# princeton-nlp/DensePhrases

Hardware: NVIDIA H100
Metric: queries/sec top-10 over PQ96 phrase index (higher is better)
Workload: dtype f32

## Files before the change

### densephrases_b200/csrc/common.cuh

```cuda
#pragma once
#include <cuda_runtime.h>
#include <stdint.h>
#include <stdio.h>
#include <string>

#define DPH_D 768
#define DPH_M 96
#define DPH_KSUB 256
#define DPH_DSUB 8
#define DPH_CODE 96
#define DPH_BLK_VECS 32
#define DPH_BLK_BYTES 3072
#define DPH_NEUTRAL (-3.402823466e+38f)

#define DPH_API extern "C" __attribute__((visibility("default")))
void dph_set_error(const std::string& msg);

#define DPH_CUDA(call)                                                                              \
    do {                                                                                            \
        cudaError_t e__ = (call);                                                                   \
        if (e__ != cudaSuccess) {                                                                   \
            dph_set_error(std::string(#call) + ": " + cudaGetErrorString(e__) + " @" + __FILE__ + ":" + \
                          std::to_string(__LINE__));                                                \
            return 1;                                                                               \
        }                                                                                           \
    } while (0)
#define DPH_CHECK(cond, msg)                                                        \
    do {                                                                            \
        if (!(cond)) { dph_set_error(std::string(msg) + " (" #cond ")"); return 1; } \
    } while (0)
#define DPH_TRY(call)            \
    do {                         \
        int r__ = (call);        \
        if (r__) return r__;     \
    } while (0)

struct DphPerDeviceOnce {
    bool done[64] = {};
    bool first() {
        int d = 0;
        cudaGetDevice(&d);
        d &= 63;
        if (done[d]) return false;
        done[d] = true;
        return true;
    }
};

__device__ __forceinline__ float2 dph_ffma2(float2 a, float2 b, float2 c) { return make_float2(fmaf(a.x, b.x, c.x), fmaf(a.y, b.y, c.y)); }
__device__ __forceinline__ float2 dph_fadd2(float2 a, float2 b) { return make_float2(__fadd_rn(a.x, b.x), __fadd_rn(a.y, b.y)); }

__host__ __device__ __forceinline__ uint64_t dph_mix64(uint64_t x) {
    x += 0x9E3779B97F4A7C15ull;
    x = (x ^ (x >> 30)) * 0xBF58476D1CE4E5B9ull;
    x = (x ^ (x >> 27)) * 0x94D049BB133111EBull;
    return x ^ (x >> 31);
}
__host__ __device__ __forceinline__ uint64_t dph_rnd64(uint64_t seed, uint64_t stream, uint64_t a, uint64_t b) {
    return dph_mix64(dph_mix64(dph_mix64(seed ^ (stream * 0xA24BAED4963EE407ull)) + a) + b);
}
__host__ __device__ __forceinline__ float dph_approx_normal(uint64_t u, float sigma_over_std) {
    int32_t s = (int32_t)(u & 0xFFFF) + (int32_t)((u >> 16) & 0xFFFF) + (int32_t)((u >> 32) & 0xFFFF) + (int32_t)(u >> 48) - 131070;
    return (float)s * sigma_over_std;
}
#define DPH_IH4_STD 37837.227f
enum { DPH_STREAM_CODES = 1, DPH_STREAM_CENTROIDS = 2, DPH_STREAM_PQ = 3 };

__host__ __device__ __forceinline__ uint32_t dph_fkey(float f) {
    uint32_t b;
#ifdef __CUDA_ARCH__
    b = __float_as_uint(f);
#else
    memcpy(&b, &f, 4);
#endif
    return (b & 0x80000000u) ? ~b : (b | 0x80000000u);
}
__host__ __device__ __forceinline__ float dph_fkey_inv(uint32_t k) {
    uint32_t b = (k & 0x80000000u) ? (k & 0x7FFFFFFFu) : ~k;
#ifdef __CUDA_ARCH__
    return __uint_as_float(b);
#else
    float f; memcpy(&f, &b, 4); return f;
#endif
}
__host__ __device__ __forceinline__ uint64_t dph_ckey(float score, uint32_t gidx) {
    return ((uint64_t)dph_fkey(score) << 32) | (uint64_t)(0xFFFFFFFFu - gidx);
}
__host__ __device__ __forceinline__ float dph_ckey_score(uint64_t k) { return dph_fkey_inv((uint32_t)(k >> 32)); }
__host__ __device__ __forceinline__ uint32_t dph_ckey_gidx(uint64_t k) { return 0xFFFFFFFFu - (uint32_t)k; }

__host__ __device__ __forceinline__ int dph_blk_addr(int lane, int m) {
    int seg = m >> 5, s = ((m & 31) - lane) & 31;
    int t = seg * 32 + s;
    return (t >> 4) * 512 + lane * 16 + (t & 15);
}

struct __align__(16) DphSeg {
    long long blk;
    int len;
    unsigned gstart;
    float dis0;
    unsigned wrel;
    unsigned wend;
    int list;
};

struct DphWork {
    long long total_blocks;
};
struct DphPairWork {
    long long total_blocks;
    long long per;
    int total_units;
    int next_unit;
};
struct __align__(16) DphUnit {
    long long blk;
    int len;
    unsigned bi0, bend;
    int nq;
    int list, pad;
    unsigned q[4];
    unsigned gs[4];
    float base[4];
    float step[4];
};
#define DPH_PAIR_SEG_MIN 128
#define DPH_PAIR_UNITS_PER_CTA 16
```

### densephrases_b200/csrc/index.cu

```cuda
#include "index_internal.cuh"
#include <algorithm>
#include <numeric>
#include <stdlib.h>
#include <string.h>
#include <thrust/device_ptr.h>
#include <thrust/execution_policy.h>
#include <thrust/sequence.h>
#include <thrust/sort.h>

static thread_local std::string g_err;
void dph_set_error(const std::string& msg) { g_err = msg; }
DPH_API const char* dph_last_error(void) { return g_err.c_str(); }
DPH_API int dph_version(void) { return 103; }
int g_dph_tune[8] = {1, 0, 0, 0, 0, 0, 0, 0};
DPH_API int dph_set_tuning(int knob, int value) {
    DPH_CHECK(knob >= 0 && knob < 8, "dph_set_tuning: unknown knob");
    g_dph_tune[knob] = value;
    return 0;
}

int DevBuf::ensure(size_t bytes) {
    if (bytes <= cap) return 0;
    if (p) cudaFree(p);
    p = nullptr; cap = 0;
// ... 298 lines not shown
    if (l < lo || l >= hi) { dm_ids[dm0 + r] = 0x7FFFFFFFFFFFFFFFll; dm_rows[dm0 + r] = -1; return; }
    const long long j = (long long)len_old[l] + (s - bstart[l]);
    const long long blk = boff_new[l] + (j >> 5);
    const int lane = (int)(j & 31);
    uint4 row4[6];
#pragma unroll
    for (int c = 0; c < 6; c++) row4[c] = reinterpret_cast<const uint4*>(codes_all + r * DPH_CODE)[c];
    dph_store_row(codes_new, blk, lane, reinterpret_cast<const unsigned char*>(row4));
    const long long id = ids_all[r];
    ids_new[blk * 32 + lane] = id;
    dm_ids[dm0 + r] = id;
    dm_rows[dm0 + r] = blk * 32 + lane;
}

DPH_API int dph_index_add_with_ids(dph_index* ix, const float* x, int64_t n, const int64_t* ids, int mem) {
    DPH_TRY(check_ready(ix, 1));
    DPH_CHECK(n >= 0, "add_with_ids: n must be >= 0");
    DPH_CUDA(cudaSetDevice(ix->device));
    if (n == 0) return 0;
    cudaStream_t st = ix->stream;
    const int64_t nlist = ix->nlist, lo = ix->list_lo, hi = ix->list_hi;
    for (float& a : ix->add_ms) a = 0.f;
    DevTmp tmp;
    const char* oom = "add_with_ids: not enough device memory for the batch; the index is unchanged";
    int64_t *list_all, *ids_all; uint8_t* codes_all; int *flag, *cnt;
    DPH_TRY(tmp.alloc(&list_all, n, oom)); DPH_TRY(tmp.alloc(&ids_all, n, oom)); DPH_TRY(tmp.alloc(&codes_all, (size_t)n * DPH_M, oom));
    DPH_TRY(tmp.alloc(&flag, 1, oom)); DPH_TRY(tmp.alloc(&cnt, nlist, oom));
    DPH_CUDA(cudaMemsetAsync(flag, 0, 4, st));
    DPH_CUDA(cudaMemsetAsync(cnt, 0, nlist * 4, st));
    if (mem == DPH_MEM_DEVICE) DPH_TRY(dph_encode_rows(ix, x, n, list_all, codes_all, flag));
    else {
        const int64_t cs = std::min(dph_encode_chunk(ix), n);
        DPH_TRY(ix->xdev.ensure((size_t)cs * ix->d * 4));
        for (int64_t o = 0; o < n; o += cs) {
            const int64_t m = std::min(cs, n - o);
            DPH_CUDA(cudaMemcpyAsync(ix->xdev.p, x + o * ix->d, (size_t)m * ix->d * 4, cudaMemcpyHostToDevice, st));
            DPH_TRY(dph_encode_rows(ix, ix->xdev.as<float>(), m, list_all + o, codes_all + o * DPH_M, flag));
        }
    }
    if (ids) DPH_CUDA(cudaMemcpyAsync(ids_all, ids, (size_t)n * 8, mem == DPH_MEM_HOST ? cudaMemcpyHostToDevice : cudaMemcpyDeviceToDevice, st));
    else iota_kernel<<<(unsigned)((n + 255) / 256), 256, 0, st>>>((long long*)ids_all, n, ix->ntotal);
    add_validate_kernel<<<(unsigned)((n + 255) / 256), 256, 0, st>>>((const long long*)list_all, (const long long*)ids_all, n, flag, cnt);
    DPH_CUDA(cudaGetLastError());
    int h_flag = 0;
    std::vector<int32_t> h_cnt(nlist);
    DPH_CUDA(cudaMemcpyAsync(&h_flag, flag, 4, cudaMemcpyDeviceToHost, st));
    DPH_CUDA(cudaMemcpyAsync(h_cnt.data(), cnt, nlist * 4, cudaMemcpyDeviceToHost, st));
    DPH_CUDA(cudaStreamSynchronize(st));
    DPH_CHECK(!(h_flag & 1), "add_with_ids: the input holds a non-finite value; the index is unchanged");
    DPH_CHECK(!(h_flag & 2), "add_with_ids: negative label (-1 marks padding rows); the index is unchanged");
    DPH_CHECK(!(h_flag & 4), "add_with_ids: a vector has no best list; the index is unchanged");

    std::vector<int64_t> len_new(nlist), start_new(nlist + 1, 0), boff_new(nlist, -1), bstart(nlist, 0), lrs_old(std::max<int64_t>(hi - lo, 1), 0);
    std::vector<int32_t> len32(nlist);
    int64_t nb = 0, rows = 0, rows_old = 0, in_shard = 0;
    for (int64_t l = 0; l < nlist; l++) {
        len_new[l] = ix->h_list_len[l] + h_cnt[l];
        DPH_CHECK(len_new[l] < (1ll << 31), "add_with_ids: a list would exceed 2^31 - 1 rows; the index is unchanged");
        len32[l] = (int32_t)len_new[l];
        start_new[l + 1] = start_new[l] + len_new[l];
        if (l + 1 < nlist) bstart[l + 1] = bstart[l] + h_cnt[l];
    }
    for (int64_t l = lo; l < hi; l++) {
        boff_new[l] = nb; lrs_old[l - lo] = rows_old;
        nb += (len_new[l] + 31) / 32; rows += len_new[l]; rows_old += ix->h_list_len[l]; in_shard += h_cnt[l];
    }
    const bool was_explicit = ix->ids != nullptr;
    const int64_t dm_old = was_explicit ? ix->dm_n : ix->ntotal_local;
    const int64_t dm_cap = dm_old + n;

    const char* oom2 = "add_with_ids: not enough device memory for the re-layout (the old and the new code buffers of the shard are live "
                       "together); the index is unchanged";
    uint8_t* codes_new; int64_t *ids_new, *dm_ids_new, *dm_rows_new, *d_boff_new, *d_bstart, *d_lrs, *perm;
    DPH_TRY(tmp.alloc(&codes_new, (size_t)nb * DPH_BLK_BYTES, oom2)); DPH_TRY(tmp.alloc(&ids_new, (size_t)nb * 32, oom2));
    DPH_TRY(tmp.alloc(&dm_ids_new, dm_cap, oom2)); DPH_TRY(tmp.alloc(&dm_rows_new, dm_cap, oom2));
    DPH_TRY(tmp.alloc(&d_boff_new, nlist, oom2)); DPH_TRY(tmp.alloc(&d_bstart, nlist, oom2));
    DPH_TRY(tmp.alloc(&d_lrs, lrs_old.size(), oom2)); DPH_TRY(tmp.alloc(&perm, n, oom2));
    DPH_CUDA(cudaMemcpyAsync(d_boff_new, boff_new.data(), nlist * 8, cudaMemcpyHostToDevice, st));
    DPH_CUDA(cudaMemcpyAsync(d_bstart, bstart.data(), nlist * 8, cudaMemcpyHostToDevice, st));
    DPH_CUDA(cudaMemcpyAsync(d_lrs, lrs_old.data(), lrs_old.size() * 8, cudaMemcpyHostToDevice, st));

    const bool prof = ix->profile && ix->aev[0];
    if (prof) DPH_CUDA(cudaEventRecord(ix->aev[4], st));
    const long long *bo_new = (const long long*)d_boff_new, *bo_old = (const long long*)ix->blk_off;
    if (nb > 0) {
        relayout_codes_kernel<<<(unsigned)nb, 192, 0, st>>>(codes_new, 0, bo_new, bo_old, ix->list_len, lo, hi, ix->codes);
        relayout_ids_kernel<<<(unsigned)nb, 32, 0, st>>>((long long*)ids_new, 0, bo_new, bo_old, ix->list_len, lo, hi, (const long long*)ix->ids,
                                                       (const long long*)ix->list_start, (const long long*)d_lrs, (long long*)dm_ids_new,
                                                       (long long*)dm_rows_new);
    }
    if (was_explicit && ix->dm_n > 0)
        remap_dm_kernel<<<(unsigned)((ix->dm_n + 255) / 256), 256, 0, st>>>((const long long*)ix->dm_ids, (const long long*)ix->dm_rows, ix->dm_n,
                                                                           bo_old, bo_new, lo, hi, (long long*)dm_ids_new, (long long*)dm_rows_new);
    DPH_CUDA(cudaGetLastError());
    try {
        thrust::device_ptr<long long> kp((long long*)list_all), pp((long long*)perm);
        thrust::sequence(thrust::cuda::par.on(st), pp, pp + n);
        thrust::stable_sort_by_key(thrust::cuda::par.on(st), kp, kp + n, pp);
        add_scatter_kernel<<<(unsigned)((n + 127) / 128), 128, 0, st>>>(n, (const long long*)list_all, (const long long*)perm, (const long long*)d_bstart,
                                                                       ix->list_len, bo_new, lo, hi, codes_all, (const long long*)ids_all, codes_new,
                                                                       (long long*)ids_new, (long long*)dm_ids_new, (long long*)dm_rows_new, dm_old);
        DPH_CUDA(cudaGetLastError());
        thrust::device_ptr<long long> dk((long long*)dm_ids_new), dv((long long*)dm_rows_new);
        thrust::stable_sort_by_key(thrust::cuda::par.on(st), dk, dk + dm_cap, dv);
    } catch (const std::exception& e) {
        cudaGetLastError();
        dph_set_error(std::string("add_with_ids: device sort failed; the index is unchanged: ") + e.what());
        return 1;
    }
    if (prof) DPH_CUDA(cudaEventRecord(ix->aev[5], st));
    DPH_CUDA(cudaStreamSynchronize(st));

    DPH_CUDA(cudaMemcpy(ix->blk_off, d_boff_new, nlist * 8, cudaMemcpyDeviceToDevice));
    DPH_CUDA(cudaMemcpy(ix->list_len, len32.data(), nlist * 4, cudaMemcpyHostToDevice));
    DPH_CUDA(cudaMemcpy(ix->list_start, start_new.data(), (nlist + 1) * 8, cudaMemcpyHostToDevice));
    const int64_t nb_old = ix->blk_cap < 0 ? ix->nblocks_local : ix->blk_cap;
    int64_t old_bytes = std::max<int64_t>(nb_old * DPH_BLK_BYTES, 1);
    if (ix->ids) old_bytes += std::max<int64_t>(nb_old * 32, 1) * 8;
    if (ix->dm_ids) old_bytes += 2 * std::max<int64_t>(ix->dm_cap < 0 ? ix->ntotal_local : ix->dm_cap, 1) * 8;
    const int64_t new_bytes = std::max<int64_t>(nb * DPH_BLK_BYTES, 1) + std::max<int64_t>(nb * 32, 1) * 8 + 2 * std::max<int64_t>(dm_cap, 1) * 8;
    void* olds[] = {ix->codes, ix->ids, ix->dm_ids, ix->dm_rows};
    for (void* p : olds) if (p) cudaFree(p);
    ix->codes = codes_new; ix->ids = ids_new; ix->dm_ids = dm_ids_new; ix->dm_rows = dm_rows_new;
    for (void* p : {(void*)codes_new, (void*)ids_new, (void*)dm_ids_new, (void*)dm_rows_new}) tmp.release(p);
    ix->bytes += new_bytes - old_bytes;
    ix->dm_n = dm_old + in_shard; ix->dm_cap = dm_cap;
    ix->h_list_len = len_new; ix->h_list_start = start_new;
    ix->ntotal = start_new[nlist]; ix->ntotal_local = rows; ix->nblocks_local = nb; ix->blk_cap = -1;
    if (prof) DPH_CUDA(cudaEventElapsedTime(&ix->add_ms[3], ix->aev[4], ix->aev[5]));
    return 0;
}

__global__ void __launch_bounds__(192) read_blocks_kernel(const uint8_t* codes, long long nblocks, const long long* blk_off, const int* list_len,
                                                          long long list_lo, long long list_hi, const long long* ids, const long long* list_start,
                                                          const long long* local_row_start, long long blk0, long long raw_row0, uint8_t* raw,
                                                          long long* raw_ids) {
    const long long blk = blk0 + blockIdx.x;
    if (blk >= nblocks) return;
    const int lane = threadIdx.x & 31, c = threadIdx.x >> 5;
    __shared__ long long s_l;
    if (threadIdx.x == 0) s_l = list_of_block(blk_off, list_lo, list_hi, blk);
    __syncthreads();
    const long long l = s_l;
    const long long j = (blk - blk_off[l]) * 32 + lane;
    if (j >= (long long)list_len[l]) return;
    const long long row = local_row_start[l - list_lo] + j - raw_row0;
    const uint4 v = *reinterpret_cast<const uint4*>(codes + blk * DPH_BLK_BYTES + c * 512 + lane * 16);
    unsigned char bytes[16];
    memcpy(bytes, &v, 16);
    const int seg = c >> 1;
#pragma unroll
    for (int b = 0; b < 16; b++) { const int t = c * 16 + b; raw[row * DPH_CODE + seg * 32 + ((lane + (t & 31)) & 31)] = bytes[b]; }
    if (c == 0 && raw_ids) raw_ids[row] = ids ? ids[blk * 32 + lane] : list_start[l] + j;
}

DPH_API int dph_index_copy_lists(dph_index* ix, uint8_t* codes_out, int64_t* ids_out) {
    DPH_CHECK(ix && ix->list_len, "copy_lists: lists are not set");
    DPH_CUDA(cudaSetDevice(ix->device));
    const int64_t lo = ix->list_lo, hi = ix->list_hi;
    const std::vector<int64_t>& len = ix->h_list_len;
    if (ix->ntotal_local == 0) return 0;
    std::vector<int64_t> boff(hi - lo), lrs(hi - lo);
    for (int64_t l = lo, nb = 0, rows = 0; l < hi; l++) { boff[l - lo] = nb; lrs[l - lo] = rows; nb += (len[l] + 31) / 32; rows += len[l]; }
    const int64_t chunk_rows = dph_chunk_rows();
    auto chunk_end = [&](int64_t l0, int64_t& acc) {
        int64_t l1 = l0;
        acc = 0;
        while (l1 < hi && (acc == 0 || acc + len[l1] <= chunk_rows)) { acc += len[l1]; l1++; }
        return l1;
    };
    int64_t max_rows = 0;
    for (int64_t l0 = lo, acc = 0; l0 < hi;) { const int64_t l1 = chunk_end(l0, acc); max_rows = std::max(max_rows, acc); l0 = l1; }
    DevTmp tmp;
    uint8_t* d_raw; int64_t *d_ids, *d_lrs;
    DPH_TRY(tmp.alloc(&d_raw, (size_t)max_rows * DPH_CODE, "copy_lists: staging"));
    DPH_TRY(tmp.alloc(&d_ids, (size_t)max_rows, "copy_lists: staging"));
    DPH_TRY(tmp.alloc(&d_lrs, lrs.size(), "copy_lists: staging"));
    DPH_CUDA(cudaMemcpyAsync(d_lrs, lrs.data(), lrs.size() * 8, cudaMemcpyHostToDevice, ix->stream));
    for (int64_t l0 = lo; l0 < hi;) {
        int64_t acc = 0;
        const int64_t l1 = chunk_end(l0, acc);
        const int64_t r0 = lrs[l0 - lo], b0 = boff[l0 - lo], b1 = l1 < hi ? boff[l1 - lo] : ix->nblocks_local;
        if (acc > 0 && b1 > b0) {
            read_blocks_kernel<<<(unsigned)(b1 - b0), 192, 0, ix->stream>>>(ix->codes, b1, (const long long*)ix->blk_off, ix->list_len, lo, hi,
                                                                           (const long long*)ix->ids, (const long long*)ix->list_start,
                                                                           (const long long*)d_lrs, b0, r0, d_raw, ids_out ? (long long*)d_ids : nullptr);
            DPH_CUDA(cudaGetLastError());
            DPH_CUDA(cudaMemcpyAsync(codes_out + (size_t)r0 * DPH_CODE, d_raw, (size_t)acc * DPH_CODE, cudaMemcpyDeviceToHost, ix->stream));
            if (ids_out) DPH_CUDA(cudaMemcpyAsync(ids_out + r0, d_ids, (size_t)acc * 8, cudaMemcpyDeviceToHost, ix->stream));
            DPH_CUDA(cudaStreamSynchronize(ix->stream));
        }
        l0 = l1;
    }
    return 0;
}

DPH_API int dph_index_get_list_len(const dph_index* ix, int64_t* list_len_out) {
    DPH_CHECK(ix && ix->list_len, "lists are not set");
    std::copy(ix->h_list_len.begin(), ix->h_list_len.end(), list_len_out);
    return 0;
}
DPH_API int dph_index_last_add_ms(const dph_index* ix, float* ms_out) {
    DPH_CHECK(ix->aev[0] != nullptr, "profiling was never enabled");
    std::copy(ix->add_ms, ix->add_ms + 4, ms_out);
    return 0;
}

DPH_API int64_t dph_index_ntotal(const dph_index* ix) { return ix->ntotal; }
DPH_API int64_t dph_index_ntotal_local(const dph_index* ix) { return ix->ntotal_local; }
DPH_API int dph_index_d(const dph_index* ix) { return ix->d; }
DPH_API int64_t dph_index_nlist(const dph_index* ix) { return ix->nlist; }
DPH_API int dph_index_nprobe(const dph_index* ix) { return ix->nprobe; }
DPH_API int dph_index_set_nprobe(dph_index* ix, int nprobe) {
    DPH_CHECK(nprobe >= 1 && nprobe <= DPH_MAX_NPROBE, "nprobe must be in [1,1024]");
    ix->nprobe = nprobe;
    return 0;
}
DPH_API int dph_index_set_coarse_tc(dph_index* ix, int on) { ix->coarse_tc = on ? 1 : 0; return 0; }
DPH_API int dph_index_set_scan_mode(dph_index* ix, int mode) {
    DPH_CHECK(mode >= 0 && mode <= 4, "bad scan mode");
    ix->scan_mode = mode;
    return 0;
}
DPH_API int dph_index_get_opq(const dph_index* ix, float* A_out, int mem) {
    DPH_CHECK(ix->A != nullptr, "OPQ matrix not set");
    DPH_CUDA(cudaMemcpy(A_out, ix->A, (size_t)ix->d * ix->d * 4, mem == DPH_MEM_HOST ? cudaMemcpyDeviceToHost : cudaMemcpyDeviceToDevice));
    return 0;
}
DPH_API int dph_index_set_profile(dph_index* ix, int on) {
    DPH_CUDA(cudaSetDevice(ix->device));
    if (on && !ix->ev0[0])
        for (int i = 0; i < DPH_PROF_RING; i++) { DPH_CUDA(cudaEventCreate(&ix->ev0[i])); DPH_CUDA(cudaEventCreate(&ix->ev1[i])); }
    if (on && !ix->aev[0])
        for (cudaEvent_t& e : ix->aev) DPH_CUDA(cudaEventCreate(&e));
    ix->profile = on != 0;
    ix->prof_n = 0;
    return 0;
}
DPH_API int dph_index_last_scan_ms(dph_index* ix, float* ms) {
    DPH_CHECK(ix->ev0[0] && ix->prof_n > 0, "no profiled search");
    int i = (int)((ix->prof_n - 1) % DPH_PROF_RING);
    DPH_CUDA(cudaEventSynchronize(ix->ev1[i]));
    DPH_CUDA(cudaEventElapsedTime(ms, ix->ev0[i], ix->ev1[i]));
    return 0;
}
DPH_API int dph_index_profile_scan_ms(dph_index* ix, float* ms_out, int max_out) {
    DPH_CHECK(ix->ev0[0] != nullptr, "profiling was never enabled");
    int n = (int)std::min<int64_t>(std::min<int64_t>(ix->prof_n, DPH_PROF_RING), max_out);
    for (int j = 0; j < n; j++) {
        int i = (int)((ix->prof_n - n + j) % DPH_PROF_RING);
        DPH_CUDA(cudaEventSynchronize(ix->ev1[i]));
        DPH_CUDA(cudaEventElapsedTime(ms_out + j, ix->ev0[i], ix->ev1[i]));
    }
    return n < 0 ? 0 : 0 * n;
}
DPH_API int dph_index_profile_count(const dph_index* ix) { return (int)std::min<int64_t>(ix->prof_n, DPH_PROF_RING); }
DPH_API int64_t dph_index_device_bytes(const dph_index* ix) { return ix->bytes; }
DPH_API const int32_t* dph_index_last_flags(const dph_index* ix) { return ix->flags.as<int32_t>(); }
DPH_API const int32_t* dph_index_last_probes(const dph_index* ix) { return ix->key.as<int32_t>(); }
DPH_API const float* dph_index_last_coarse(const dph_index* ix) { return ix->cd.as<float>(); }
DPH_API const float* dph_index_last_xr(const dph_index* ix) { return ix->xr.as<float>(); }
DPH_API int dph_index_last_used_pair_mode(const dph_index* ix) { return ix->last_group > 1 ? 1 : 0; }
DPH_API int dph_index_last_group_size(const dph_index* ix) { return ix->last_group; }
DPH_API int dph_index_copy_last(dph_index* ix, int which, void* dst_host, int64_t bytes) {
    const void* src = which == 0 ? ix->flags.p : which == 1 ? ix->key.p : which == 2 ? ix->cd.p : which == 3 ? ix->xr.p : nullptr;
    DPH_CHECK(src != nullptr, "copy_last: nothing to copy");
    DPH_CUDA(cudaStreamSynchronize(ix->stream));
    DPH_CUDA(cudaMemcpy(dst_host, src, (size_t)bytes, cudaMemcpyDeviceToHost));
    return 0;
}

static int search_chunk(dph_index* ix, const float* x_dev, int64_t n, int k, float* D, int64_t* I, uint32_t* G, int stage = 0,
                        unsigned long long* keys64 = nullptr) {
    cudaStream_t st = ix->stream;
    const int nprobe = ix->nprobe;
    const int grid = ix->num_sms;
    const int keep_single = k + DPH_KEEP_SLACK;
    const int keep_pair = k + (k / 2 > DPH_KEEP_SLACK ? k / 2 : DPH_KEEP_SLACK);
    const int keep_quad = k + (2 * k > 100 ? 2 * k : 100);
    const int keep_max = keep_quad > keep_pair ? keep_quad : keep_pair;
    DPH_TRY(ix->xr.ensure((size_t)n * ix->d * 4));
    DPH_TRY(ix->S.ensure((size_t)n * ix->nlist * 4));
    DPH_TRY(ix->key.ensure((size_t)n * nprobe * 4));
    DPH_TRY(ix->cd.ensure((size_t)n * nprobe * 4));
    DPH_TRY(ix->lut_canon.ensure((size_t)n * DPH_LUT_CANON_FLOATS * 4));
    DPH_TRY(ix->lutmax.ensure((size_t)n * DPH_M * 4));
    DPH_TRY(ix->segs.ensure((size_t)n * nprobe * sizeof(DphSeg)));
    DPH_TRY(ix->wpre.ensure((size_t)(n + 1) * 8));
    DPH_TRY(ix->qinfo.ensure((size_t)n * 4));
    DPH_TRY(ix->eps.ensure((size_t)n * 4));
    DPH_TRY(ix->nseg.ensure((size_t)n * 4));
    const int64_t eff_probe = std::min<int64_t>(nprobe, ix->nlist);
    const int64_t nl_local = std::max<int64_t>(ix->list_hi - ix->list_lo, 1);
    const bool long_lists = ix->ntotal_local / nl_local >= 4096;
    const bool shared = long_lists && n * eff_probe * 2 >= ix->nlist * 3;
    int group = 1;
    if (ix->scan_mode == DPH_SCAN_PAIR) group = 2;
    else if (ix->scan_mode == DPH_SCAN_QUAD) group = 4;
    else if (ix->scan_mode == DPH_SCAN_FAST && shared) group = 4;
    if (group == 4 && keep_quad > DPH_QUAD_KEEP_MAX) group = 2;
    if (group == 2 && keep_pair > 1536 - DPH_SCAN_THREADS) group = 1;
    const bool pair = group > 1;
    const int keep_fast = group == 4 ? keep_quad : (group == 2 ? keep_pair : keep_single);
    DPH_TRY(ix->cand.ensure(((size_t)(2 * grid + 2 * n + 2) + (pair ? (size_t)(n * nprobe + 2 * DPH_PAIR_UNITS_PER_CTA * grid + 2 * n + 16) : 0)) * keep_max * 8));
    DPH_TRY(ix->cand_off.ensure((size_t)(n + 1) * 8));
    DPH_TRY(ix->cand_cnt.ensure((size_t)n * 4));
    DPH_TRY(ix->gthr.ensure((size_t)n * 4));
    DPH_TRY(ix->flags.ensure((size_t)n * 4));
    DPH_TRY(ix->work.ensure(sizeof(DphWork)));
    DPH_TRY(ix->lutmin.ensure((size_t)n * DPH_M * 4));
    DPH_TRY(ix->lutmaxv.ensure((size_t)n * DPH_M * 4));
    if (pair) {
        DPH_TRY(ix->lutq.ensure((size_t)n * DPH_LUT_SCAN_FLOATS * 2));
        DPH_TRY(ix->qparams.ensure((size_t)n * 8));
        DPH_TRY(ix->gdense.ensure((size_t)n * nprobe * 4));
        DPH_TRY(ix->pl_cnt.ensure((size_t)ix->nlist * 4));
        DPH_TRY(ix->pl_fill.ensure((size_t)ix->nlist * 4));
        DPH_TRY(ix->pl_off.ensure((size_t)(ix->nlist + 1) * 4));
        DPH_TRY(ix->pl_blockpre.ensure((size_t)(ix->nlist + 1) * 8));
        DPH_TRY(ix->pl_entries.ensure((size_t)n * nprobe * 4));
        DPH_TRY(ix->pl_unitpre.ensure((size_t)(ix->nlist + 1) * 4));
        DPH_TRY(ix->pl_units.ensure((size_t)(n * nprobe + DPH_PAIR_UNITS_PER_CTA * grid + 16) * 8));
        if (group == 4) DPH_TRY(ix->pl_udesc.ensure((size_t)(n * nprobe + DPH_PAIR_UNITS_PER_CTA * grid + 16) * sizeof(DphUnit)));
        DPH_TRY(ix->pairwork.ensure(sizeof(DphPairWork)));
    }
    ix->last_n = n;
    if (stage != 1 && stage != 3) ix->last_group = group;
    if (stage == 1) ix->last_coarse_n = n;

    if (stage == 1) {
        const int64_t nl = ix->list_hi - ix->list_lo;
        DPH_TRY(dph_launch_sgemm_nt_seq(x_dev, n, ix->A, ix->d, ix->d, ix->xr.as<float>(), st));
        if (ix->coarse_tc) {
            int rc = dph_coarse_tc(ix, n, ix->list_lo, nl, nprobe, keys64, nullptr, nullptr, st);
            if (rc == 0) return 0;
            if (rc != 1) return rc;
        }
        DPH_TRY(dph_launch_sgemm_nt_seq(ix->xr.as<float>(), n, ix->C + ix->list_lo * ix->d, nl, ix->d, ix->S.as<float>(), st));
        DPH_TRY(dph_launch_coarse_select(ix->S.as<float>(), n, nl, nprobe, nullptr, nullptr, st, keys64, (unsigned)ix->list_lo));
        return 0;
    }
    if (stage == 0 || stage == 3) {
        DPH_TRY(dph_launch_sgemm_nt_seq(x_dev, n, ix->A, ix->d, ix->d, ix->xr.as<float>(), st));
        int rc = ix->coarse_tc ? dph_coarse_tc(ix, n, 0, ix->nlist, nprobe, nullptr, ix->key.as<int32_t>(), ix->cd.as<float>(), st) : 1;
        if (rc > 1) return rc;
        if (rc == 1) {
            DPH_TRY(dph_launch_sgemm_nt_seq(ix->xr.as<float>(), n, ix->C, ix->nlist, ix->d, ix->S.as<float>(), st));
            DPH_TRY(dph_launch_coarse_select(ix->S.as<float>(), n, ix->nlist, nprobe, ix->key.as<int32_t>(), ix->cd.as<float>(), st, nullptr, 0u, nullptr, 0,
                                             &ix->selkeys));
        }
        if (stage == 3) return 0;
    }
    DPH_TRY(dph_launch_lut(ix->xr.as<float>(), n, ix->pq, ix->lut_canon.as<float>(), ix->lutmax.as<float>(),
                           ix->lutmin.as<float>(), ix->lutmaxv.as<float>(), pair ? ix->lutq.p : nullptr,
                           pair ? ix->qparams.as<float2>() : nullptr, st, group));
    if (ix->scan_mode != DPH_SCAN_EXACT) {
        DPH_TRY(dph_launch_plan(ix, n, k, keep_fast, grid, nullptr, st, group));
        if (ix->profile) DPH_CUDA(cudaEventRecord(ix->ev0[ix->prof_n % DPH_PROF_RING], st));
        if (pair) DPH_TRY(dph_launch_scan_pair(ix, n, keep_fast, grid, st, group));
        else DPH_TRY(dph_launch_scan(ix, n, k, keep_fast, DPH_SCAN_FAST, grid, st));
        if (ix->profile) { DPH_CUDA(cudaEventRecord(ix->ev1[ix->prof_n % DPH_PROF_RING], st)); ix->prof_n++; }
        DPH_TRY(dph_launch_merge(ix, n, k, DPH_SCAN_FAST, nullptr, D, I, G, st));
        DPH_TRY(dph_launch_plan(ix, n, k, k, grid, ix->flags.as<int32_t>(), st, 1));
        DPH_TRY(dph_launch_scan(ix, n, k, k, DPH_SCAN_EXACT, grid, st));
        DPH_TRY(dph_launch_merge(ix, n, k, DPH_SCAN_EXACT, ix->flags.as<int32_t>(), D, I, G, st));
    } else {
        DPH_CUDA(cudaMemsetAsync(ix->flags.p, 0, (size_t)n * 4, st));
        DPH_TRY(dph_launch_plan(ix, n, k, k, grid, nullptr, st, 1));
        if (ix->profile) DPH_CUDA(cudaEventRecord(ix->ev0[ix->prof_n % DPH_PROF_RING], st));
        DPH_TRY(dph_launch_scan(ix, n, k, k, DPH_SCAN_EXACT, grid, st));
        if (ix->profile) { DPH_CUDA(cudaEventRecord(ix->ev1[ix->prof_n % DPH_PROF_RING], st)); ix->prof_n++; }
        DPH_TRY(dph_launch_merge(ix, n, k, DPH_SCAN_EXACT, nullptr, D, I, G, st));
    }
    return 0;
}

static int check_ready(dph_index* ix, int k) {
    DPH_CHECK(ix && ix->A && ix->C && ix->pq && ix->list_len, "index is not fully constructed (opq/centroids/pq/lists)");
    DPH_CHECK(k >= 1 && k <= DPH_MAX_K, "k must be in [1,1024]");
    return 0;
}
static int64_t chunk_size(const dph_index* ix, int64_t n) {
    int64_t c = (1ll << 28) / std::max<int64_t>(ix->nlist, 1);
    c = std::max<int64_t>(1, std::min<int64_t>(c, 4096));
    return std::min(c, n);
}

DPH_API int dph_index_search_partial(dph_index* ix, const float* x_dev, int64_t n, int k, float* D, int64_t* I, uint32_t* G) {
    DPH_TRY(check_ready(ix, k));
    DPH_CUDA(cudaSetDevice(ix->device));
    const int64_t cs = chunk_size(ix, n);
    for (int64_t o = 0; o < n; o += cs) {
        int64_t m = std::min(cs, n - o);
        DPH_TRY(search_chunk(ix, x_dev + o * ix->d, m, k, D + o * k, I + o * k, G + o * k));
    }
    return 0;
}

DPH_API int dph_index_coarse_local(dph_index* ix, const float* x_dev, int64_t n, uint64_t* keys_dev) {
    DPH_TRY(check_ready(ix, 1));
    DPH_CUDA(cudaSetDevice(ix->device));
    DPH_CHECK(n <= chunk_size(ix, n), "coarse_local: batch too large for one chunk");
    return search_chunk(ix, x_dev, n, 1, nullptr, nullptr, nullptr, 1, (unsigned long long*)keys_dev);
}
DPH_API int dph_index_search_preassigned(dph_index* ix, const uint64_t* keys_gathered_dev, int nshards, int64_t n, int k, float* D_dev,
                                         int64_t* I_dev, uint32_t* G_dev) {
    DPH_TRY(check_ready(ix, k));
    DPH_CUDA(cudaSetDevice(ix->device));
    DPH_CHECK(n == ix->last_coarse_n, "search_preassigned must follow coarse_local with the same batch");
    DPH_TRY(ix->key.ensure((size_t)n * ix->nprobe * 4));
    DPH_TRY(ix->cd.ensure((size_t)n * ix->nprobe * 4));
    DPH_TRY(dph_launch_coarse_merge((const unsigned long long*)keys_gathered_dev, nshards, n, ix->nprobe, ix->key.as<int32_t>(), ix->cd.as<float>(),
                                    ix->stream));
    return search_chunk(ix, nullptr, n, k, D_dev, I_dev, G_dev, 2, nullptr);
}

__global__ void pack_records_kernel(const float* __restrict__ xr, const int* __restrict__ key, const float* __restrict__ cd, int nprobe, float* __restrict__ rec) {
    const long long q = blockIdx.x;
    const int R = DPH_D + 2 * nprobe;
    float* o = rec + q * R;
    for (int t = threadIdx.x; t < R; t += blockDim.x)
        o[t] = t < DPH_D ? xr[q * DPH_D + t] : (t < DPH_D + nprobe ? __int_as_float(key[q * nprobe + t - DPH_D]) : cd[q * nprobe + t - DPH_D - nprobe]);
}
__global__ void unpack_records_kernel(const float* __restrict__ rec, int nprobe, float* __restrict__ xr, int* __restrict__ key, float* __restrict__ cd) {
    const long long q = blockIdx.x;
    const int R = DPH_D + 2 * nprobe;
    const float* r = rec + q * R;
    for (int t = threadIdx.x; t < R; t += blockDim.x) {
        const float v = r[t];
        if (t < DPH_D) xr[q * DPH_D + t] = v;
        else if (t < DPH_D + nprobe) key[q * nprobe + t - DPH_D] = __float_as_int(v);
        else cd[q * nprobe + t - DPH_D - nprobe] = v;
    }
}
DPH_API int dph_index_record_floats(const dph_index* ix) { return ix->d + 2 * ix->nprobe; }
DPH_API int dph_index_coarse_split(dph_index* ix, const float* x_dev, int64_t n_local, float* rec_dev) {
    DPH_TRY(check_ready(ix, 1));
    DPH_CUDA(cudaSetDevice(ix->device));
    if (n_local == 0) return 0;
    DPH_CHECK(n_local <= chunk_size(ix, n_local), "coarse_split: slice too large for one chunk");
    DPH_TRY(search_chunk(ix, x_dev, n_local, 1, nullptr, nullptr, nullptr, 3, nullptr));
    pack_records_kernel<<<(unsigned)n_local, 256, 0, ix->stream>>>(ix->xr.as<float>(), ix->key.as<int>(), ix->cd.as<float>(), ix->nprobe, rec_dev);
    DPH_CUDA(cudaGetLastError());
    return 0;
}
DPH_API int dph_index_search_assigned(dph_index* ix, const float* rec_dev, int64_t n, int k, float* D_dev, int64_t* I_dev, uint32_t* G_dev) {
    DPH_TRY(check_ready(ix, k));
    DPH_CUDA(cudaSetDevice(ix->device));
    if (n == 0) return 0;
    DPH_TRY(ix->xr.ensure((size_t)n * ix->d * 4));
    DPH_TRY(ix->key.ensure((size_t)n * ix->nprobe * 4));
    DPH_TRY(ix->cd.ensure((size_t)n * ix->nprobe * 4));
    unpack_records_kernel<<<(unsigned)n, 256, 0, ix->stream>>>(rec_dev, ix->nprobe, ix->xr.as<float>(), ix->key.as<int>(), ix->cd.as<float>());
    DPH_CUDA(cudaGetLastError());
    return search_chunk(ix, nullptr, n, k, D_dev, I_dev, G_dev, 2, nullptr);
}

DPH_API int dph_index_search(dph_index* ix, const float* x, int64_t n, int k, float* D, int64_t* I, int mem) {
    DPH_TRY(check_ready(ix, k));
    DPH_CUDA(cudaSetDevice(ix->device));
    if (n == 0) return 0;
    DPH_TRY(ix->Gp.ensure((size_t)n * k * 4));
    if (mem == DPH_MEM_DEVICE) return dph_index_search_partial(ix, x, n, k, D, I, ix->Gp.as<uint32_t>());
    DPH_TRY(ix->xdev.ensure((size_t)n * ix->d * 4));
    DPH_TRY(ix->Dp.ensure((size_t)n * k * 4));
    DPH_TRY(ix->Ip.ensure((size_t)n * k * 8));
    DPH_CUDA(cudaMemcpyAsync(ix->xdev.p, x, (size_t)n * ix->d * 4, cudaMemcpyHostToDevice, ix->stream));
    DPH_TRY(dph_index_search_partial(ix, ix->xdev.as<float>(), n, k, ix->Dp.as<float>(), ix->Ip.as<int64_t>(), ix->Gp.as<uint32_t>()));
    DPH_CUDA(cudaMemcpyAsync(D, ix->Dp.p, (size_t)n * k * 4, cudaMemcpyDeviceToHost, ix->stream));
    DPH_CUDA(cudaMemcpyAsync(I, ix->Ip.p, (size_t)n * k * 8, cudaMemcpyDeviceToHost, ix->stream));
    DPH_CUDA(cudaStreamSynchronize(ix->stream));
    return 0;
}

struct LocateArgs {
    const long long* list_start; long long nlist; long long list_lo, list_hi; const long long* blk_off; const int* list_len;
    const long long* dm_ids; const long long* dm_rows; long long dm_n; bool explicit_ids;
};
__device__ __forceinline__ bool locate_label(const LocateArgs& a, long long id, long long& l, long long& prow) {
    if (!a.explicit_ids) {
        if (id < 0 || id >= a.list_start[a.nlist]) return false;
        long long lo = 0, hi = a.nlist;
        while (hi - lo > 1) { long long mid = (lo + hi) >> 1; if (a.list_start[mid] <= id) lo = mid; else hi = mid; }
        l = lo;
        if (l < a.list_lo || l >= a.list_hi) return false;
        long long j = id - a.list_start[l];
        prow = (a.blk_off[l] + (j >> 5)) * 32 + (j & 31);
        return true;
    }
    long long lo = 0, hi = a.dm_n;
    if (hi == 0) return false;
    while (hi - lo > 1) { long long mid = (lo + hi) >> 1; if (a.dm_ids[mid] <= id) lo = mid; else hi = mid; }
    if (a.dm_ids[lo] != id) return false;
    prow = a.dm_rows[lo];
    l = list_of_block(a.blk_off, a.list_lo, a.list_hi, prow >> 5);
    return true;
}

__global__ void __launch_bounds__(96) reconstruct_kernel(LocateArgs la, const long long* ids, long long m, const uint8_t* codes, const float* C,
                                                          const float* pq, float* out, unsigned char* found) {
    const long long i = blockIdx.x;
    const int t = threadIdx.x;
    __shared__ long long s_l, s_prow; __shared__ int s_ok;
    if (t == 0) { long long l = 0, pr = 0; s_ok = locate_label(la, ids[i], l, pr) ? 1 : 0; s_l = l; s_prow = pr; }
    __syncthreads();
    float4* o = reinterpret_cast<float4*>(out + i * DPH_D + t * 8);
    if (!s_ok) { o[0] = make_float4(0, 0, 0, 0); o[1] = make_float4(0, 0, 0, 0); if (t == 0 && found) found[i] = 0; return; }
    const long long blk = s_prow >> 5; const int lane = (int)(s_prow & 31);
    const unsigned char code = codes[blk * DPH_BLK_BYTES + dph_blk_addr(lane, t)];
    const float4* cb = reinterpret_cast<const float4*>(pq + ((size_t)t * 256 + code) * 8);
    const float4* ce = reinterpret_cast<const float4*>(C + s_l * DPH_D + t * 8);
    float4 a0 = cb[0], a1 = cb[1], c0 = ce[0], c1 = ce[1];
    o[0] = make_float4(a0.x + c0.x, a0.y + c0.y, a0.z + c0.z, a0.w + c0.w);
    o[1] = make_float4(a1.x + c1.x, a1.y + c1.y, a1.z + c1.z, a1.w + c1.w);
    if (t == 0 && found) found[i] = 1;
}

static LocateArgs make_locate(const dph_index* ix) {
    LocateArgs la;
    la.list_start = (const long long*)ix->list_start; la.nlist = ix->nlist; la.list_lo = ix->list_lo; la.list_hi = ix->list_hi;
    la.blk_off = (const long long*)ix->blk_off; la.list_len = ix->list_len; la.dm_ids = (const long long*)ix->dm_ids;
    la.dm_rows = (const long long*)ix->dm_rows; la.dm_n = ix->dm_n; la.explicit_ids = ix->ids != nullptr;
    return la;
}

DPH_API int dph_index_reconstruct_batch(dph_index* ix, const int64_t* ids, int64_t m, float* out, uint8_t* found, int mem) {
    DPH_TRY(check_ready(ix, 1));
    DPH_CUDA(cudaSetDevice(ix->device));
    if (m == 0) return 0;
    const int64_t* d_ids = ids; float* d_out = out; uint8_t* d_found = found;
    DevBuf &tmp_ids = ix->rb_ids, &tmp_out = ix->rb_out, &tmp_found = ix->rb_found;
    if (mem == DPH_MEM_HOST) {
        DPH_TRY(tmp_ids.ensure((size_t)m * 8)); DPH_TRY(tmp_out.ensure((size_t)m * ix->d * 4)); DPH_TRY(tmp_found.ensure((size_t)m));
        DPH_CUDA(cudaMemcpyAsync(tmp_ids.p, ids, (size_t)m * 8, cudaMemcpyHostToDevice, ix->stream));
        d_ids = tmp_ids.as<int64_t>(); d_out = tmp_out.as<float>(); d_found = tmp_found.as<uint8_t>();
    }
    reconstruct_kernel<<<(unsigned)m, 96, 0, ix->stream>>>(make_locate(ix), (const long long*)d_ids, m, ix->codes, ix->C, ix->pq, d_out, d_found);
    DPH_CUDA(cudaGetLastError());
    if (mem == DPH_MEM_HOST) {
        DPH_CUDA(cudaMemcpyAsync(out, d_out, (size_t)m * ix->d * 4, cudaMemcpyDeviceToHost, ix->stream));
        if (found) DPH_CUDA(cudaMemcpyAsync(found, d_found, (size_t)m, cudaMemcpyDeviceToHost, ix->stream));
        DPH_CUDA(cudaStreamSynchronize(ix->stream));
    }
    return 0;
}

__global__ void __launch_bounds__(96) window_scores_kernel(LocateArgs la, const float* __restrict__ xq, const long long* __restrict__ first_id,
                                                            int L, const uint8_t* __restrict__ codes, const float* __restrict__ C,
                                                            const float* __restrict__ pq, float* __restrict__ out) {
    const long long i = blockIdx.x;
    const int t = threadIdx.x, lane = t & 31, warp = t >> 5;
    __shared__ long long s_l, s_prow; __shared__ int s_ok; __shared__ float red[3];
    const float4* xp = reinterpret_cast<const float4*>(xq + i * DPH_D + t * 8);
    const float4 x0 = xp[0], x1 = xp[1];
    for (int w = 0; w < L; w++) {
        if (t == 0) { long long l = 0, pr = 0; s_ok = locate_label(la, first_id[i] + w, l, pr) ? 1 : 0; s_l = l; s_prow = pr; }
        __syncthreads();
        float part = 0.f;
        if (s_ok) {
            const long long blk = s_prow >> 5; const int ln = (int)(s_prow & 31);
            const unsigned char code = codes[blk * DPH_BLK_BYTES + dph_blk_addr(ln, t)];
            const float4* cb = reinterpret_cast<const float4*>(pq + ((size_t)t * 256 + code) * 8);
            const float4* ce = reinterpret_cast<const float4*>(C + s_l * DPH_D + t * 8);
            const float4 a0 = cb[0], a1 = cb[1], c0 = ce[0], c1 = ce[1];
            part = fmaf(x0.x, a0.x + c0.x, part); part = fmaf(x0.y, a0.y + c0.y, part); part = fmaf(x0.z, a0.z + c0.z, part); part = fmaf(x0.w, a0.w + c0.w, part);
            part = fmaf(x1.x, a1.x + c1.x, part); part = fmaf(x1.y, a1.y + c1.y, part); part = fmaf(x1.z, a1.z + c1.z, part); part = fmaf(x1.w, a1.w + c1.w, part);
        }
#pragma unroll
        for (int off = 16; off > 0; off >>= 1) part += __shfl_xor_sync(0xffffffffu, part, off);
        if (lane == 0) red[warp] = part;
        __syncthreads();
        if (t == 0) out[i * L + w] = (red[0] + red[1]) + red[2];
        __syncthreads();
    }
}

DPH_API int dph_index_window_scores(dph_index* ix, const float* q, const int64_t* first_id, int64_t m, int L, float* out_scores, int mem) {
    DPH_TRY(check_ready(ix, 1));
    DPH_CHECK(L >= 1 && L <= 64, "window length out of range");
    DPH_CUDA(cudaSetDevice(ix->device));
    if (m == 0) return 0;
    DevBuf &tq = ix->ws_q, &tid = ix->ws_id, &tout = ix->ws_out, &txq = ix->ws_xq;
    const float* dq = q; const int64_t* did = first_id; float* dout = out_scores;
    if (mem == DPH_MEM_HOST) {
        DPH_TRY(tq.ensure((size_t)m * ix->d * 4)); DPH_TRY(tid.ensure((size_t)m * 8)); DPH_TRY(tout.ensure((size_t)m * L * 4));
        DPH_CUDA(cudaMemcpyAsync(tq.p, q, (size_t)m * ix->d * 4, cudaMemcpyHostToDevice, ix->stream));
        DPH_CUDA(cudaMemcpyAsync(tid.p, first_id, (size_t)m * 8, cudaMemcpyHostToDevice, ix->stream));
        dq = tq.as<float>(); did = tid.as<int64_t>(); dout = tout.as<float>();
    }
    DPH_TRY(txq.ensure((size_t)m * ix->d * 4));
    DPH_TRY(dph_launch_sgemm_nt_seq(dq, m, ix->A, ix->d, ix->d, txq.as<float>(), ix->stream));
    window_scores_kernel<<<(unsigned)m, 96, 0, ix->stream>>>(make_locate(ix), txq.as<float>(), (const long long*)did, L, ix->codes, ix->C, ix->pq, dout);
    DPH_CUDA(cudaGetLastError());
    if (mem == DPH_MEM_HOST) DPH_CUDA(cudaMemcpyAsync(out_scores, dout, (size_t)m * L * 4, cudaMemcpyDeviceToHost, ix->stream));
    if (mem == DPH_MEM_HOST) DPH_CUDA(cudaStreamSynchronize(ix->stream));
    return 0;
}
```

### densephrases_b200/csrc/index_internal.cuh

```cuda
#pragma once
#include "common.cuh"
#include "../../include/dph_b200.h"
#include <algorithm>
#include <string.h>
#include <vector>

#define DPH_SCAN_THREADS 512
#define DPH_SCAN_WARPS (DPH_SCAN_THREADS / 32)
#define DPH_CAND_CAP 3072
#define DPH_PAIR_CAP 1280
#define DPH_QUAD_KEEP_MAX 256

#define DPH_KEEP_SLACK 32
#define DPH_MAX_K 1024
#define DPH_PROF_RING 64
#define DPH_MAX_NPROBE 1024
#define DPH_SURV_CAP 2048
#define DPH_LUT_SCAN_FLOATS (3 * 256 * 64)
#define DPH_LUT_CANON_FLOATS (96 * 256)
#define DPH_LUTC_IDX(m, code) ((((m) >> 5) << 13) + ((code) << 5) + ((m) & 31))
#define DPH_SEG_SMEM 256
#define DPH_L2_PREFETCH_ROUNDS 4

struct DevBuf {
    void* p = nullptr;
    size_t cap = 0;
    int ensure(size_t bytes);
    void release();
    template <class T> T* as() const { return (T*)p; }
};

struct dph_index {
    int device = 0;
    int d = DPH_D, M = DPH_M;
    int64_t nlist = 0;
    int nprobe = 256;
    int scan_mode = DPH_SCAN_FAST;
    cudaStream_t stream = 0;
    int num_sms = 132;

    float* A = nullptr;
    float* C = nullptr;
    float* pq = nullptr;
    int64_t list_lo = 0, list_hi = 0;
    int64_t ntotal = 0, ntotal_local = 0, nblocks_local = 0;
    int32_t* list_len = nullptr;
    int64_t* list_start = nullptr;
    int64_t* blk_off = nullptr;
    uint8_t* codes = nullptr;
    int64_t* ids = nullptr;
    int64_t* dm_ids = nullptr;
    int64_t* dm_rows = nullptr;
    int64_t dm_n = 0;
    int64_t dm_cap = -1;
    std::vector<int64_t> h_list_len;
    std::vector<int64_t> h_list_start;
    int64_t bytes = 0;

    DevBuf xdev, xr, S, key, cd, lut_canon, lutmax, segs, wpre, qinfo, cand, cand_off, cand_cnt, gthr, flags,
        work, Dp, Ip, Gp, Dh, Ih, eps, nseg,
        lutmin, lutmaxv, lutq, qparams, gdense, pl_cnt, pl_fill, pl_off, pl_blockpre, pl_entries, pl_unitpre, pl_units, pl_udesc, pairwork,
        csplit, xsplit, candkeys, cflags, selkeys, recbuf,
        rb_ids, rb_out, rb_found, ws_q, ws_id, ws_out, ws_xq,
        enc_key, enc_cd, enc_list, enc_codes;
    int64_t csplit_lo = -1, csplit_nl = -1;
    int coarse_tc = 1;
    int64_t last_n = 0;
    int last_group = 1;
    int64_t last_coarse_n = -1;
    bool profile = false;
    cudaEvent_t ev0[DPH_PROF_RING] = {}, ev1[DPH_PROF_RING] = {};
    int64_t prof_n = 0;
    cudaEvent_t aev[6] = {};
    float add_ms[4] = {};
    float remove_ms[3] = {};
    float train_ms[3] = {};
    int64_t remove_tmp_peak = 0;
    int64_t blk_cap = -1;
};

__device__ __forceinline__ long long list_of_block(const long long* blk_off, long long lo, long long hi, long long blk) {
    while (hi - lo > 1) { long long mid = (lo + hi) >> 1; if (blk_off[mid] <= blk) lo = mid; else hi = mid; }
    return lo;
}
__device__ __forceinline__ void dph_store_row(uint8_t* codes, long long blk, int lane, const unsigned char* row) {
#pragma unroll
    for (int c = 0; c < 6; c++) {
        unsigned char bytes[16];
        const int seg = c >> 1;
#pragma unroll
        for (int b = 0; b < 16; b++) { const int t = c * 16 + b; bytes[b] = row[seg * 32 + ((lane + (t & 31)) & 31)]; }
        uint4 v;
        memcpy(&v, bytes, 16);
        *reinterpret_cast<uint4*>(codes + blk * DPH_BLK_BYTES + c * 512 + lane * 16) = v;
    }
}
__device__ __forceinline__ void dph_load_row(const uint8_t* codes, long long blk, int lane, unsigned char* row) {
#pragma unroll
    for (int c = 0; c < 6; c++) {
        const uint4 v = *reinterpret_cast<const uint4*>(codes + blk * DPH_BLK_BYTES + c * 512 + lane * 16);
        unsigned char bytes[16];
        memcpy(bytes, &v, 16);
        const int seg = c >> 1;
#pragma unroll
        for (int b = 0; b < 16; b++) { const int t = c * 16 + b; row[seg * 32 + ((lane + (t & 31)) & 31)] = bytes[b]; }
    }
}

struct DevTmp {
    std::vector<void*> ps;
    int64_t live = 0, peak = 0;
    ~DevTmp() { for (void* p : ps) if (p) cudaFree(p); }
    template <class T> int alloc(T** out, size_t count, const char* what) {
        const size_t bytes = std::max<size_t>(count, 1) * sizeof(T);
        cudaError_t e = cudaMalloc((void**)out, bytes);
        if (e != cudaSuccess) {
            cudaGetLastError();
            *out = nullptr;
            dph_set_error(std::string(what) + ": " + cudaGetErrorString(e));
            return 1;
        }
        ps.push_back(*out);
        live += (int64_t)bytes; peak = std::max(peak, live);
        return 0;
    }
    void release(void* p) { for (void*& q : ps) if (q == p) q = nullptr; }
};

int64_t dph_chunk_rows();
__global__ void relayout_codes_kernel(uint8_t* dst, long long blk0, const long long* boff_new, const long long* boff_old, const int* len_old,
                                      long long lo, long long hi, const uint8_t* codes_old);
__global__ void relayout_ids_kernel(long long* dst, long long blk0, const long long* boff_new, const long long* boff_old, const int* len_old,
                                    long long lo, long long hi, const long long* ids_old, const long long* list_start_old,
                                    const long long* lrs_old, long long* dm_ids, long long* dm_rows);

extern int g_dph_tune[8];
int dph_launch_sgemm_nt_seq(const float* X, int64_t n, const float* W, int64_t m, int K, float* out, cudaStream_t st);
int dph_launch_coarse_select(const float* S, int64_t n, int64_t nlist, int nprobe, int32_t* key, float* cd, cudaStream_t st,
                             unsigned long long* keys64 = nullptr, unsigned list_base = 0, const int* only_rows = nullptr, int64_t ld = 0,
                             DevBuf* tmp = nullptr);
int dph_coarse_tc(dph_index* ix, int64_t n, int64_t lo, int64_t nl, int nprobe, unsigned long long* keys64, int32_t* key, float* cd, cudaStream_t st,
                  const float* xr = nullptr, const float* C = nullptr);
int dph_launch_coarse_merge(const unsigned long long* keys, int W, int64_t n, int nprobe, int32_t* key, float* cd, cudaStream_t st,
                            unsigned long long* keys64 = nullptr);
int dph_launch_lut(const float* xr, int64_t n, const float* pq, float* lut_canon, float* lutmax, float* lutmin, float* lutmaxv,
                   void* lutq, float2* qparams, cudaStream_t st, int group);
int dph_launch_plan(dph_index* ix, int64_t n, int k, int keep, int grid, const int32_t* only_flagged, cudaStream_t st, int group);
int dph_launch_scan_pair(dph_index* ix, int64_t n, int keep, int grid, cudaStream_t st, int group);
int dph_launch_scan(dph_index* ix, int64_t n, int k, int keep, int mode, int grid, cudaStream_t st);
int dph_launch_merge(dph_index* ix, int64_t n, int k, int mode, const int32_t* only_flagged, float* D, int64_t* I,
                     uint32_t* G, cudaStream_t st);
int dph_scan_setup_attrs();
int64_t dph_encode_chunk(const dph_index* ix);
int dph_encode_rows(dph_index* ix, const float* x_dev, int64_t n, int64_t* list_out, uint8_t* codes_out, int* bad);
int dph_coarse_top1(dph_index* ix, const float* xr, const float* C, int64_t n, int32_t* key, float* cd, cudaStream_t st);
int dph_pq_assign(dph_index* ix, const float* xr, const float* C, const int32_t* key, const float* pq, int64_t n, int64_t* list_out,
                  uint8_t* codes_out, cudaStream_t st);
__global__ void nonfinite_kernel(const float* __restrict__ x, long long count, int* __restrict__ bad);
```

### densephrases_b200/csrc/prep.cu

```cuda
#include "index_internal.cuh"
#include "select.cuh"

#define GBM 128
#define GBN 128
#define GBK 8
__global__ void __launch_bounds__(256) sgemm_nt_seq_kernel(const float* __restrict__ X, long long n, const float* __restrict__ W,
                                                            long long m, int K, float* __restrict__ out) {
    __shared__ __align__(16) float As[2][GBK][GBM];
    __shared__ __align__(16) float Bs[2][GBK][GBN];
    const int tid = threadIdx.x;
    const long long row0 = (long long)blockIdx.y * GBM, col0 = (long long)blockIdx.x * GBN;
    const int lr = tid & 127, lk4 = tid >> 7;
    const long long arow = row0 + lr, brow = col0 + lr;
    const bool aok = arow < n, bok = brow < m;
    const float4* ap = reinterpret_cast<const float4*>(X + (aok ? arow : 0) * K) + lk4;
    const float4* bp = reinterpret_cast<const float4*>(W + (bok ? brow : 0) * K) + lk4;
    const int tx = tid & 15, ty = tid >> 4;
    float2 acc[8][4];
#pragma unroll
    for (int i = 0; i < 8; i++)
#pragma unroll
        for (int j = 0; j < 4; j++) acc[i][j] = make_float2(0.0f, 0.0f);
    const float4 z4 = make_float4(0.f, 0.f, 0.f, 0.f);
    float4 ra = aok ? __ldg(ap) : z4, rb = bok ? __ldg(bp) : z4;
// ... 519 lines not shown
            lutmax[o] = a; lutmin[o] = lo; lutmaxv[o] = hi;
        }
    }
    const int seg = m0 >> 5, mo = m0 & 31;
    for (int qi = 0; qi < nq; qi++) {
        float* dst = lut_canon + (size_t)(q0 + qi) * DPH_LUT_CANON_FLOATS + (size_t)seg * (256 * 32) + mo;
        const float* t = tile + qi * MS * LUT_TILE_LD;
        for (int idx = j; idx < 256 * MS; idx += 256) dst[(idx / MS) * 32 + (idx % MS)] = t[(idx % MS) * LUT_TILE_LD + (idx / MS)];
    }
}

#define DPH_QMAX 682
#define DPH_QMAX8 255
template <class T, int QMAX>
__global__ void __launch_bounds__(256) lutq_kernel(const float* __restrict__ lut_canon, const float* __restrict__ lutmin,
                                                    const float* __restrict__ lutmaxv, T* __restrict__ lutq,
                                                    float2* __restrict__ qparams) {
    __shared__ float tile[256 * 33];
    __shared__ float s_min[32];
    __shared__ float s_step, s_base;
    const long long q = blockIdx.x;
    const int seg = blockIdx.y, j = threadIdx.x, lane = j & 31;
    if (j < 32) {
        float r = 0.f, b = 0.f;
        for (int m = lane; m < DPH_M; m += 32) { r = fmaxf(r, lutmaxv[q * DPH_M + m] - lutmin[q * DPH_M + m]); b += lutmin[q * DPH_M + m]; }
#pragma unroll
        for (int off = 16; off > 0; off >>= 1) { r = fmaxf(r, __shfl_xor_sync(0xffffffffu, r, off)); b += __shfl_xor_sync(0xffffffffu, b, off); }
        if (lane == 0) { s_step = fmaxf(r / (float)QMAX, 1e-30f); s_base = b; }
        s_min[lane] = lutmin[q * DPH_M + seg * 32 + lane];
    }
    const float* src = lut_canon + (size_t)q * DPH_LUT_CANON_FLOATS + (size_t)seg * (256 * 32);
    for (int idx = j; idx < 256 * 32; idx += 256) tile[(idx >> 5) * 33 + (idx & 31)] = __ldg(src + idx);
    __syncthreads();
    const float inv = 1.0f / s_step;
    T* dst = lutq + ((size_t)q * 3 + seg) * (256 * 64);
    for (int idx = j; idx < 256 * 64; idx += 256) {
        const int row = idx >> 6, w = idx & 63, ml = w & 31;
        int qv = (int)((tile[row * 33 + ml] - s_min[ml]) * inv + 0.5f);
        qv = qv < 0 ? 0 : (qv > QMAX ? QMAX : qv);
        dst[idx] = (w < 63) ? (T)qv : (T)0;
    }
    if (seg == 0 && j == 0) qparams[q] = make_float2(s_step, s_base);
}

int dph_launch_lut(const float* xr, int64_t n, const float* pq, float* lut_canon, float* lutmax, float* lutmin, float* lutmaxv,
                   void* lutq, float2* qparams, cudaStream_t st, int group) {
    if (n == 0) return 0;
    static DphPerDeviceOnce lut_once;
    constexpr int lut_smem = 4 * 32 * LUT_TILE_LD * 4;
    if (lut_once.first()) {
        DPH_CUDA(cudaFuncSetAttribute(lut_kernel<4, 32>, cudaFuncAttributeMaxDynamicSharedMemorySize, lut_smem));
        DPH_CUDA(cudaFuncSetAttribute(lut_kernel<8, 16>, cudaFuncAttributeMaxDynamicSharedMemorySize, lut_smem));
    }
    const int lv = g_dph_tune[2];
    if (lv == 2) lut_kernel<8, 16><<<dim3((unsigned)((n + 7) / 8), 6), 256, lut_smem, st>>>(xr, pq, n, lut_canon, lutmax, lutmin, lutmaxv);
    else lut_kernel<4, 32><<<dim3((unsigned)((n + 3) / 4), 3), 256, lut_smem, st>>>(xr, pq, n, lut_canon, lutmax, lutmin, lutmaxv);
    DPH_CUDA(cudaGetLastError());
    if (lutq) {
        if (group == 4) lutq_kernel<unsigned char, DPH_QMAX8><<<dim3((unsigned)n, 3), 256, 0, st>>>(lut_canon, lutmin, lutmaxv, (unsigned char*)lutq, qparams);
        else lutq_kernel<unsigned short, DPH_QMAX><<<dim3((unsigned)n, 3), 256, 0, st>>>(lut_canon, lutmin, lutmaxv, (unsigned short*)lutq, qparams);
        DPH_CUDA(cudaGetLastError());
    }
    return 0;
}

struct PlanArgs {
    const int* key; const float* cd; const int* list_len; const long long* blk_off;
    long long list_lo, list_hi; int nprobe; long long n;
    const int* only_flagged;
    const float* lutmax;
    DphSeg* segs; unsigned* qblocks; int* nseg; float* eps;
    unsigned* gdense;
    const float2* qparams;
};
__global__ void __launch_bounds__(256) plan_segs_kernel(PlanArgs a) {
    const int lane = threadIdx.x & 31;
    const long long q = (long long)blockIdx.x * 8 + (threadIdx.x >> 5);
    if (q >= a.n) return;
    const bool active = a.only_flagged ? (a.only_flagged[q] != 0) : true;
    if (!active) {
        if (lane == 0) { a.qblocks[q] = 0u; a.nseg[q] = 0; }
        return;
    }
    unsigned gacc = 0, wacc = 0;
    int sacc = 0;
    float dmax = 0.0f;
    for (int r0 = 0; r0 < a.nprobe; r0 += 32) {
        const int r = r0 + lane;
        int l = -1, len = 0; float d0 = 0.0f; unsigned nb = 0; long long blk = -1;
        if (r < a.nprobe) {
            l = a.key[q * a.nprobe + r];
            d0 = a.cd[q * a.nprobe + r];
            if (l >= 0) {
                len = a.list_len[l];
                dmax = fmaxf(dmax, fabsf(d0));
                if (active && len > 0 && l >= a.list_lo && l < a.list_hi) { nb = (unsigned)((len + 31) >> 5); blk = a.blk_off[l]; }
            }
        }
        unsigned gl = (unsigned)len, wl = nb;
#pragma unroll
        for (int off = 1; off < 32; off <<= 1) {
            unsigned g2 = __shfl_up_sync(0xffffffffu, gl, off), w2 = __shfl_up_sync(0xffffffffu, wl, off);
            if (lane >= off) { gl += g2; wl += w2; }
        }
        if (a.gdense && r < a.nprobe) a.gdense[q * a.nprobe + r] = gacc + gl - (unsigned)len;
        const unsigned have = __ballot_sync(0xffffffffu, nb > 0);
        if (nb > 0) {
            DphSeg s;
            s.blk = blk; s.len = len; s.gstart = gacc + gl - (unsigned)len; s.dis0 = d0;
            s.wrel = wacc + wl - nb; s.wend = wacc + wl; s.list = l;
            a.segs[q * a.nprobe + sacc + __popc(have & ((1u << lane) - 1u))] = s;
        }
        sacc += __popc(have);
        gacc += __shfl_sync(0xffffffffu, gl, 31);
        wacc += __shfl_sync(0xffffffffu, wl, 31);
    }
#pragma unroll
    for (int off = 16; off > 0; off >>= 1) dmax = fmaxf(dmax, __shfl_xor_sync(0xffffffffu, dmax, off));
    float lsum = 0.0f;
    for (int m = lane; m < DPH_M; m += 32) lsum += a.lutmax[q * DPH_M + m];
#pragma unroll
    for (int off = 16; off > 0; off >>= 1) lsum += __shfl_xor_sync(0xffffffffu, lsum, off);
    if (lane == 0) {
        a.qblocks[q] = wacc;
        a.nseg[q] = sacc;
        const float gamma96 = 5.7221e-6f;
        float e = 2.0f * gamma96 * (dmax + lsum) * 1.01f;
        if (a.qparams) e += 96.0f * 0.502f * a.qparams[q].x + 8e-6f * (dmax + lsum);
        a.eps[q] = e;
    }
}

struct PlanScanArgs {
    const unsigned* qblocks; long long n; int keep; int grid;
    long long* qpre; long long* cand_off; int* cand_cnt; unsigned* gthr; DphWork* work;
    const DphPairWork* pairwork; const int* nseg;
};
__global__ void __launch_bounds__(1024) plan_scan_kernel(PlanScanArgs a) {
    __shared__ long long wsum[32];
    __shared__ long long carry, total;
    const int tid = threadIdx.x, lane = tid & 31, warp = tid >> 5;
    if (tid == 0) carry = 0;
    __syncthreads();
    for (long long base = 0; base < a.n; base += 1024) {
        long long q = base + tid;
        long long v = q < a.n ? (long long)a.qblocks[q] : 0, incl = v;
#pragma unroll
        for (int off = 1; off < 32; off <<= 1) { long long t = __shfl_up_sync(0xffffffffu, incl, off); if (lane >= off) incl += t; }
        if (lane == 31) wsum[warp] = incl;
        __syncthreads();
        if (warp == 0) {
            long long w = wsum[lane], wi = w;
#pragma unroll
            for (int off = 1; off < 32; off <<= 1) { long long t = __shfl_up_sync(0xffffffffu, wi, off); if (lane >= off) wi += t; }
            wsum[lane] = wi - w;
        }
        __syncthreads();
        long long excl = carry + wsum[warp] + incl - v;
        if (q < a.n) { a.qpre[q] = excl; a.cand_cnt[q] = 0; a.gthr[q] = 0u; }
        __syncthreads();
        if (tid == 1023) carry = excl + v;
        __syncthreads();
    }
    if (tid == 0) { total = carry; a.qpre[a.n] = carry; a.work->total_blocks = carry; carry = 0; }
    __syncthreads();
    const long long T = total;
    const long long per = a.pairwork ? a.pairwork->per : (T / a.grid > 0 ? T / a.grid : 1);
    for (long long base = 0; base < a.n; base += 1024) {
        long long q = base + tid;
        long long v = 0;
        if (q < a.n) {
            long long qb = (long long)a.qblocks[q];
            if (qb > 0) {
                long long parts = qb / per + 2;
                if (a.pairwork) parts = (long long)a.nseg[q] + qb / per + 1;
                else if (parts > a.grid) parts = a.grid;
                v = parts * a.keep;
            }
        }
        long long incl = v;
#pragma unroll
        for (int off = 1; off < 32; off <<= 1) { long long t = __shfl_up_sync(0xffffffffu, incl, off); if (lane >= off) incl += t; }
        if (lane == 31) wsum[warp] = incl;
        __syncthreads();
        if (warp == 0) {
            long long w = wsum[lane], wi = w;
#pragma unroll
            for (int off = 1; off < 32; off <<= 1) { long long t = __shfl_up_sync(0xffffffffu, wi, off); if (lane >= off) wi += t; }
            wsum[lane] = wi - w;
        }
        __syncthreads();
        long long excl = carry + wsum[warp] + incl - v;
        if (q < a.n) a.cand_off[q] = excl;
        __syncthreads();
        if (tid == 1023) carry = excl + v;
        __syncthreads();
    }
    if (tid == 0) a.cand_off[a.n] = carry;
}

struct PairPlanArgs {
    const int* key; long long nq_probes; int nprobe; const int* list_len; long long list_lo, list_hi, nlist; int grid;
    int* cnt; int* fill; int* off; long long* blockpre; unsigned* entries; DphPairWork* work;
    int* unitpre; unsigned long long* units;
    int gsz;
    DphUnit* udesc;
    const long long* blk_off; const float* cd; const unsigned* gdense; const float2* qparams;
};
__global__ void pair_count_kernel(PairPlanArgs a) {
    const long long i = (long long)blockIdx.x * blockDim.x + threadIdx.x;
    if (i >= a.nq_probes) return;
    const int l = a.key[i];
    if (l >= a.list_lo && l < a.list_hi && a.list_len[l] > 0) atomicAdd(&a.cnt[l], 1);
}
__global__ void __launch_bounds__(1024) pair_scan_kernel(PairPlanArgs a) {
    __shared__ long long wsa[32], wsb[32];
    __shared__ long long ca, cb;
    const int tid = threadIdx.x, lane = tid & 31, warp = tid >> 5;
    if (tid == 0) { ca = 0; cb = 0; }
    __syncthreads();
    for (long long base = a.list_lo; base < a.list_hi; base += 1024) {
        const long long l = base + tid;
        long long va = 0, vb = 0;
        if (l < a.list_hi) {
            const int c = a.cnt[l];
            va = c;
            vb = (long long)((c + a.gsz - 1) / a.gsz) * (long long)((a.list_len[l] + 31) >> 5);
        }
        long long ia = va, ib = vb;
#pragma unroll
        for (int off = 1; off < 32; off <<= 1) {
            long long t1 = __shfl_up_sync(0xffffffffu, ia, off), t2 = __shfl_up_sync(0xffffffffu, ib, off);
            if (lane >= off) { ia += t1; ib += t2; }
        }
        if (lane == 31) { wsa[warp] = ia; wsb[warp] = ib; }
        __syncthreads();
        if (warp == 0) {
            long long w1 = wsa[lane], w2 = wsb[lane], i1 = w1, i2 = w2;
#pragma unroll
            for (int off = 1; off < 32; off <<= 1) {
                long long t1 = __shfl_up_sync(0xffffffffu, i1, off), t2 = __shfl_up_sync(0xffffffffu, i2, off);
                if (lane >= off) { i1 += t1; i2 += t2; }
            }
            wsa[lane] = i1 - w1; wsb[lane] = i2 - w2;
        }
        __syncthreads();
        const long long ea = ca + wsa[warp] + ia - va, eb = cb + wsb[warp] + ib - vb;
        if (l < a.list_hi) { a.off[l] = (int)ea; a.blockpre[l] = eb; }
        __syncthreads();
        if (tid == 1023) { ca = ea + va; cb = eb + vb; }
        __syncthreads();
    }
    __shared__ long long segb_s;
    if (tid == 0) {
        a.off[a.list_hi] = (int)ca; a.blockpre[a.list_hi] = cb;
        long long segb = (cb + (long long)a.grid * DPH_PAIR_UNITS_PER_CTA - 1) / ((long long)a.grid * DPH_PAIR_UNITS_PER_CTA);
        if (segb < DPH_PAIR_SEG_MIN) segb = DPH_PAIR_SEG_MIN;
        a.work->total_blocks = cb;
        a.work->per = segb;
        segb_s = segb; ca = 0;
    }
    __syncthreads();
    const long long segb = segb_s;
    for (long long base = a.list_lo; base < a.list_hi; base += 1024) {
        const long long l = base + tid;
        long long va = 0;
        if (l < a.list_hi) {
            const long long nb = (a.list_len[l] + 31) >> 5;
            va = (long long)((a.cnt[l] + a.gsz - 1) / a.gsz) * ((nb + segb - 1) / segb);
        }
        long long ia = va;
#pragma unroll
        for (int off = 1; off < 32; off <<= 1) { long long t1 = __shfl_up_sync(0xffffffffu, ia, off); if (lane >= off) ia += t1; }
        if (lane == 31) wsa[warp] = ia;
        __syncthreads();
        if (warp == 0) {
            long long w1 = wsa[lane], i1 = w1;
#pragma unroll
            for (int off = 1; off < 32; off <<= 1) { long long t1 = __shfl_up_sync(0xffffffffu, i1, off); if (lane >= off) i1 += t1; }
            wsa[lane] = i1 - w1;
        }
        __syncthreads();
        const long long ea = ca + wsa[warp] + ia - va;
        if (l < a.list_hi) a.unitpre[l] = (int)ea;
        __syncthreads();
        if (tid == 1023) ca = ea + va;
        __syncthreads();
    }
    if (tid == 0) { a.work->total_units = (int)ca; a.work->next_unit = 0; }
}
__global__ void pair_units_kernel(PairPlanArgs a) {
    const long long l = a.list_lo + (long long)blockIdx.x * blockDim.x + threadIdx.x;
    if (l >= a.list_hi) return;
    const int cnt = a.cnt[l];
    const int items = (cnt + a.gsz - 1) / a.gsz;
    if (items == 0) return;
    const long long segb = a.work->per, nb = (a.list_len[l] + 31) >> 5;
    const int nsegs = (int)((nb + segb - 1) / segb);
    const long long u0 = a.unitpre[l];
    for (int it = 0; it < items; it++) {
        DphUnit d;
        if (a.udesc) {
            d.blk = a.blk_off[l]; d.len = a.list_len[l]; d.list = (int)l; d.pad = 0;
            d.nq = min(4, cnt - 4 * it);
            const int e0 = a.off[l] + 4 * it;
#pragma unroll
            for (int i = 0; i < 4; i++) {
                const unsigned e = a.entries[e0 + (i < d.nq ? i : 0)];
                const long long q = e >> 10; const int r = (int)(e & 1023u);
                const float2 pp = a.qparams[q];
                d.q[i] = (unsigned)q; d.gs[i] = a.gdense[q * a.nprobe + r];
                d.base[i] = a.cd[q * a.nprobe + r] + pp.y; d.step[i] = pp.x;
            }
        }
        for (int s = 0; s < nsegs; s++) {
            const long long u = u0 + (long long)s * items + it;
            a.units[u] = (unsigned long long)l | ((unsigned long long)it << 32) | ((unsigned long long)s << 48);
            if (a.udesc) {
                d.bi0 = (unsigned)(s * segb);
                d.bend = (unsigned)((nb - (long long)d.bi0 < segb) ? nb : (long long)d.bi0 + segb);
                a.udesc[u] = d;
            }
        }
    }
}
__global__ void pair_fill_kernel(PairPlanArgs a) {
    const long long i = (long long)blockIdx.x * blockDim.x + threadIdx.x;
    if (i >= a.nq_probes) return;
    const int l = a.key[i];
    if (l >= a.list_lo && l < a.list_hi && a.list_len[l] > 0) {
        const int pos = a.off[l] + atomicAdd(&a.fill[l], 1);
        a.entries[pos] = (unsigned)((i / a.nprobe) << 10) | (unsigned)(i % a.nprobe);
    }
}

int dph_launch_plan(dph_index* ix, int64_t n, int k, int keep, int grid, const int32_t* only_flagged, cudaStream_t st, int group) {
    const bool pair = group > 1;
    (void)k;
    if (n == 0) return 0;
    PlanArgs a;
    a.key = ix->key.as<int>(); a.cd = ix->cd.as<float>(); a.list_len = ix->list_len; a.blk_off = (const long long*)ix->blk_off;
    a.list_lo = ix->list_lo; a.list_hi = ix->list_hi; a.nprobe = ix->nprobe; a.n = n; a.only_flagged = only_flagged;
    a.lutmax = ix->lutmax.as<float>(); a.segs = ix->segs.as<DphSeg>(); a.qblocks = ix->qinfo.as<unsigned>(); a.nseg = ix->nseg.as<int>(); a.eps = ix->eps.as<float>();
    a.gdense = pair ? ix->gdense.as<unsigned>() : nullptr; a.qparams = pair ? ix->qparams.as<float2>() : nullptr;
    plan_segs_kernel<<<(unsigned)((n + 7) / 8), 256, 0, st>>>(a);
    DPH_CUDA(cudaGetLastError());
    if (pair) {
        PairPlanArgs p;
        p.key = ix->key.as<int>(); p.nq_probes = n * ix->nprobe; p.nprobe = ix->nprobe; p.list_len = ix->list_len; p.list_lo = ix->list_lo;
        p.list_hi = ix->list_hi; p.nlist = ix->nlist; p.grid = grid; p.cnt = ix->pl_cnt.as<int>(); p.fill = ix->pl_fill.as<int>();
        p.off = ix->pl_off.as<int>(); p.blockpre = ix->pl_blockpre.as<long long>(); p.entries = ix->pl_entries.as<unsigned>();
        p.work = ix->pairwork.as<DphPairWork>(); p.unitpre = ix->pl_unitpre.as<int>(); p.units = ix->pl_units.as<unsigned long long>();
        p.gsz = group;
        p.udesc = group == 4 ? ix->pl_udesc.as<DphUnit>() : nullptr;
        p.blk_off = (const long long*)ix->blk_off; p.cd = ix->cd.as<float>(); p.gdense = ix->gdense.as<unsigned>(); p.qparams = ix->qparams.as<float2>();
        DPH_CUDA(cudaMemsetAsync(p.cnt, 0, (size_t)ix->nlist * 4, st));
        DPH_CUDA(cudaMemsetAsync(p.fill, 0, (size_t)ix->nlist * 4, st));
        const unsigned nb = (unsigned)((p.nq_probes + 255) / 256);
        pair_count_kernel<<<nb, 256, 0, st>>>(p);
        pair_scan_kernel<<<1, 1024, 0, st>>>(p);
        pair_fill_kernel<<<nb, 256, 0, st>>>(p);
        if (ix->list_hi > ix->list_lo) pair_units_kernel<<<(unsigned)((ix->list_hi - ix->list_lo + 255) / 256), 256, 0, st>>>(p);
        DPH_CUDA(cudaGetLastError());
    }
    PlanScanArgs b;
    b.pairwork = pair ? ix->pairwork.as<DphPairWork>() : nullptr; b.nseg = ix->nseg.as<int>();
    b.qblocks = ix->qinfo.as<unsigned>(); b.n = n; b.keep = keep; b.grid = grid; b.qpre = ix->wpre.as<long long>();
    b.cand_off = ix->cand_off.as<long long>(); b.cand_cnt = ix->cand_cnt.as<int>(); b.gthr = ix->gthr.as<unsigned>();
    b.work = ix->work.as<DphWork>();
    plan_scan_kernel<<<1, 1024, 0, st>>>(b);
    DPH_CUDA(cudaGetLastError());
    return 0;
}

DPH_API int dph_sgemm_nt_seq(const float* X, int64_t n, const float* W, int64_t m, int64_t K, float* out, void* cuda_stream) {
    return dph_launch_sgemm_nt_seq(X, n, W, m, (int)K, out, (cudaStream_t)cuda_stream);
}
```

### densephrases_b200/csrc/scan.cu

```cuda
#include "index_internal.cuh"
#include "select.cuh"

struct ScanArgs {
    const uint8_t* codes; const long long* qpre; const DphSeg* segs; const int* nseg; const DphWork* work;
    const float* lut_canon;
    unsigned* gthr; unsigned long long* cand; const long long* cand_off; int* cand_cnt;
    long long n; int nprobe; int keep;
};

#define NT DPH_SCAN_THREADS
#define NW DPH_SCAN_WARPS
#define SMEM_LUT_FAST (DPH_LUT_SCAN_FLOATS * 4)
#define SMEM_LUT_EXACT (DPH_LUT_CANON_FLOATS * 4 + NW * DPH_BLK_BYTES)

struct ScanShared {
    unsigned long long cbuf[DPH_CAND_CAP];
    DphSeg segtab[DPH_SEG_SMEM];
    SelectScratch sc;
    int cnt; unsigned thr; int base; int ndone; int ndone_snap; int pad[3];
};

__device__ __forceinline__ uint4 ldg_stream(const uint4* p) {
    uint4 r;
    asm volatile("ld.global.nc.L1::no_allocate.v4.u32 {%0,%1,%2,%3}, [%4];" : "=r"(r.x), "=r"(r.y), "=r"(r.z), "=r"(r.w) : "l"(p));
    return r;
}
__device__ __forceinline__ void l2_prefetch_block(const void* p) {
    asm volatile("cp.async.bulk.prefetch.L2.global [%0], %1;" :: "l"(p), "n"(DPH_BLK_BYTES) : "memory");
}

extern __shared__ __align__(1024) unsigned char dph_smem[];
#define DPH_DYN_SMEM_BASE 0x400

template <int IMM> __device__ __forceinline__ float lds_imm(unsigned addr) {
    float v;
    asm volatile("ld.shared.f32 %0, [%1+%2];" : "=f"(v) : "r"(addr), "n"(IMM));
    return v;
}
template <int T0> __device__ __forceinline__ void fast_word(unsigned wv, unsigned y, float2& a01, float2& a23) {
    constexpr int TB = DPH_DYN_SMEM_BASE + (T0 >> 5) * 65536 + (T0 & 31) * 4;
    const float v0 = lds_imm<TB + 0>(__byte_perm(wv, y, 0x7504));
    const float v1 = lds_imm<TB + 4>(__byte_perm(wv, y, 0x7514));
    const float v2 = lds_imm<TB + 8>(__byte_perm(wv, y, 0x7524));
    const float v3 = lds_imm<TB + 12>(__byte_perm(wv, y, 0x7534));
    a01 = dph_fadd2(a01, make_float2(v0, v1));
    a23 = dph_fadd2(a23, make_float2(v2, v3));
}
template <int C> __device__ __forceinline__ void fast_chunk(const uint4& v, unsigned y, float2& a01, float2& a23) {
    fast_word<C * 16 + 0>(v.x, y, a01, a23);
    fast_word<C * 16 + 4>(v.y, y, a01, a23);
    fast_word<C * 16 + 8>(v.z, y, a01, a23);
    fast_word<C * 16 + 12>(v.w, y, a01, a23);
}

struct SegCursor {
    int seg; unsigned wrel, wend; const uint4* base; int len; unsigned gstart; float dis0;
    __device__ __forceinline__ void init() { seg = -1; wrel = 0; wend = 0; base = nullptr; len = 0; gstart = 0; dis0 = 0.f; }
    __device__ __forceinline__ void seek(const DphSeg* __restrict__ tab, unsigned b, const uint8_t* codes) {
        if (b < wend) return;
        do { seg++; } while (b >= tab[seg].wend);
        const uint4 u0 = *reinterpret_cast<const uint4*>(tab + seg);
        const uint4 u1 = *(reinterpret_cast<const uint4*>(tab + seg) + 1);
        base = reinterpret_cast<const uint4*>(codes + (long long)(((unsigned long long)u0.y << 32) | u0.x) * DPH_BLK_BYTES);
        len = (int)u0.z; gstart = u0.w; dis0 = __uint_as_float(u1.x); wrel = u1.y; wend = u1.z;
    }
    __device__ __forceinline__ const uint4* ptr(unsigned b) const { return base + (size_t)(b - wrel) * (DPH_BLK_BYTES / 16); }
};

__device__ __forceinline__ void block_compact(ScanShared* sh, int keep, unsigned* gthr_q) {
    const int tid = threadIdx.x;
    const int n = sh->cnt;
    unsigned long long* cb = sh->cbuf;
    unsigned long long pivot = block_radix_select([&](int i) { return cb[i]; }, n, keep, &sh->sc);
    unsigned long long mine[DPH_CAND_CAP / NT];
#pragma unroll
    for (int e = 0; e < DPH_CAND_CAP / NT; e++) { int i = tid + e * NT; mine[e] = (i < n) ? cb[i] : 0ull; }
    __syncthreads();
    if (tid == 0) sh->cnt = 0;
    __syncthreads();
#pragma unroll
    for (int e = 0; e < DPH_CAND_CAP / NT; e++)
        if (mine[e] >= pivot && mine[e] != 0ull) { int p = atomicAdd(&sh->cnt, 1); cb[p] = mine[e]; }
    if (tid == 0) {
        unsigned t = (unsigned)(pivot >> 32);
        unsigned old = atomicMax(gthr_q, t);
        sh->thr = t > old ? t : old;
        sh->ndone_snap = sh->ndone;
    }
    __syncthreads();
}

template <int MODE>
__global__ void __launch_bounds__(NT, 1) scan_kernel(ScanArgs a) {
    unsigned char* const smem = dph_smem;
    constexpr int LUT_BYTES = (MODE == DPH_SCAN_FAST) ? SMEM_LUT_FAST : SMEM_LUT_EXACT;
    ScanShared* sh = reinterpret_cast<ScanShared*>(smem + LUT_BYTES);
    const int tid = threadIdx.x, lane = tid & 31, warp = tid >> 5;
    const long long T = a.work->total_blocks;
    const long long G = gridDim.x, c = blockIdx.x;
    const long long g0 = T * c / G, g1 = T * (c + 1) / G;
    if (g0 >= g1) return;
    long long lo = 0, hi = a.n;
    while (hi - lo > 1) { long long mid = (lo + hi) >> 1; if (a.qpre[mid] <= g0) lo = mid; else hi = mid; }
    long long q = lo, g = g0;
    const unsigned ywin = (((unsigned)__cvta_generic_to_shared(dph_smem)) & 0xFF000000u) | ((unsigned)lane * 4u);

    while (g < g1) {
        while (a.qpre[q + 1] <= g) q++;
        const long long qstart = a.qpre[q];
        const long long gend = (a.qpre[q + 1] < g1) ? a.qpre[q + 1] : g1;
        const unsigned b0 = (unsigned)(g - qstart), b1 = (unsigned)(gend - qstart);
        __syncthreads();
        {
            const int nsg0 = a.nseg[q];
            if (nsg0 <= DPH_SEG_SMEM) {
                const uint4* src = reinterpret_cast<const uint4*>(a.segs + q * a.nprobe);
                uint4* dst = reinterpret_cast<uint4*>(sh->segtab);
                for (int i = tid; i < nsg0 * 2; i += NT) dst[i] = __ldg(src + i);
            }
        }
        if (tid == 0) { sh->cnt = 0; sh->ndone = 0; sh->ndone_snap = 0; sh->thr = *((volatile unsigned*)(a.gthr + q)); }
        __syncthreads();

        const DphSeg* tab = (a.nseg[q] <= DPH_SEG_SMEM) ? sh->segtab : (a.segs + q * a.nprobe);
        SegCursor cc, pc;
        cc.init(); pc.init();
        unsigned b = b0 + warp;
        unsigned bp = b0 + warp;
        uint4 nxt[6];
        int n_len = 0; unsigned n_gstart = 0, n_j0 = 0; float n_dis0 = 0.f;
#pragma unroll 1
        for (int r = 0; r < DPH_L2_PREFETCH_ROUNDS && bp < b1; r++, bp += NW) {
            pc.seek(tab, bp, a.codes);
            if (lane == 0) l2_prefetch_block(pc.ptr(bp));
        }
        bool more = b < b1;
        if (more) {
            cc.seek(tab, b, a.codes);
            const uint4* p = cc.ptr(b) + lane;
#pragma unroll
            for (int c6 = 0; c6 < 6; c6++) nxt[c6] = ldg_stream(p + c6 * 32);
            n_len = cc.len; n_gstart = cc.gstart; n_dis0 = cc.dis0; n_j0 = (b - cc.wrel) * 32u;
        }
        {
            const float4* src = reinterpret_cast<const float4*>(a.lut_canon + (size_t)q * DPH_LUT_CANON_FLOATS);
            constexpr int PER_T = DPH_LUT_CANON_FLOATS / 4 / NT;
            constexpr int LB = 12;
            static_assert(PER_T % LB == 0, "LUT staging batches");
            if (MODE == DPH_SCAN_FAST) {
                float* dstf = reinterpret_cast<float*>(smem);
#pragma unroll 1
                for (int i0 = tid; i0 < DPH_LUT_CANON_FLOATS / 4; i0 += NT * LB) {
                    float4 v[LB];
#pragma unroll
                    for (int e = 0; e < LB; e++) v[e] = __ldg(src + i0 + e * NT);
#pragma unroll
                    for (int e = 0; e < LB; e++) {
                        const int i = i0 + e * NT;
                        const int row = i >> 3, w = (i & 7) * 4;
                        float* r = dstf + row * 64;
                        *reinterpret_cast<float4*>(r + w) = v[e];
                        if (w < 28) *reinterpret_cast<float4*>(r + 32 + w) = v[e];
                        else { r[60] = v[e].x; r[61] = v[e].y; r[62] = v[e].z; r[63] = 0.0f; }
                    }
                }
            } else {
                float4* dst = reinterpret_cast<float4*>(smem);
#pragma unroll 8
                for (int i = tid; i < DPH_LUT_CANON_FLOATS / 4; i += NT) dst[i] = __ldg(src + i);
            }
        }
        __syncthreads();
        bool counted = false;
        while (true) {
            while (more) {
                if (*((volatile int*)&sh->cnt) > DPH_CAND_CAP - NT) break;
                uint4 cur[6];
#pragma unroll
                for (int c6 = 0; c6 < 6; c6++) cur[c6] = nxt[c6];
                const int c_len = n_len; const unsigned c_gstart = n_gstart, c_j0 = n_j0; const float c_dis0 = n_dis0;
                if (bp < b1) {
                    pc.seek(tab, bp, a.codes);
                    if (lane == 0) l2_prefetch_block(pc.ptr(bp));
                    bp += NW;
                }
                b += NW;
                more = b < b1;
                if (more) {
                    cc.seek(tab, b, a.codes);
                    const uint4* p = cc.ptr(b) + lane;
#pragma unroll
                    for (int c6 = 0; c6 < 6; c6++) nxt[c6] = ldg_stream(p + c6 * 32);
                    n_len = cc.len; n_gstart = cc.gstart; n_dis0 = cc.dis0; n_j0 = (b - cc.wrel) * 32u;
                }
                float score;
                if (MODE == DPH_SCAN_FAST) {
                    float2 a01 = make_float2(c_dis0, 0.f), a23 = make_float2(0.f, 0.f);
                    fast_chunk<0>(cur[0], ywin, a01, a23);
                    fast_chunk<1>(cur[1], ywin, a01, a23);
                    fast_chunk<2>(cur[2], ywin, a01, a23);
                    fast_chunk<3>(cur[3], ywin, a01, a23);
                    fast_chunk<4>(cur[4], ywin, a01, a23);
                    fast_chunk<5>(cur[5], ywin, a01, a23);
                    score = (a01.x + a01.y) + (a23.x + a23.y);
                } else {
                    unsigned char* stage = smem + DPH_LUT_CANON_FLOATS * 4 + warp * DPH_BLK_BYTES;
                    const float* lutc = reinterpret_cast<const float*>(smem);
#pragma unroll
                    for (int c6 = 0; c6 < 6; c6++) *reinterpret_cast<uint4*>(stage + c6 * 512 + lane * 16) = cur[c6];
                    __syncwarp();
                    float dis = c_dis0;
#pragma unroll 8
                    for (int m = 0; m < DPH_M; m++) dis += lutc[DPH_LUTC_IDX(m, (int)stage[dph_blk_addr(lane, m)])];
                    score = dis;
                    __syncwarp();
                }
                const unsigned j = c_j0 + lane;
                const unsigned sk = dph_fkey(score);
                const bool pass = ((int)j < c_len) && (sk >= *((volatile unsigned*)&sh->thr));
                const unsigned pm = __ballot_sync(0xffffffffu, pass);
                if (pm) {
                    int basep = 0;
                    if (lane == 0) basep = atomicAdd(&sh->cnt, __popc(pm));
                    basep = __shfl_sync(0xffffffffu, basep, 0);
                    if (pass) {
                        int p = basep + __popc(pm & ((1u << lane) - 1u));
                        if (p < DPH_CAND_CAP) sh->cbuf[p] = ((unsigned long long)sk << 32) | (unsigned long long)(0xFFFFFFFFu - (c_gstart + j));
                    }
                }
            }
            if (!more && !counted) { counted = true; if (lane == 0) atomicAdd(&sh->ndone, 1); }
            __syncthreads();
            if (sh->cnt > a.keep) block_compact(sh, a.keep, a.gthr + q);
            else {
                if (tid == 0) {
                    unsigned gt = *((volatile unsigned*)(a.gthr + q));
                    if (gt > sh->thr) sh->thr = gt;
                    sh->ndone_snap = sh->ndone;
                }
                __syncthreads();
            }
            if (sh->ndone_snap == NW) break;
        }
        __syncthreads();
        const int cnt = sh->cnt;
        if (tid == 0) sh->base = atomicAdd(a.cand_cnt + q, cnt);
        __syncthreads();
        {
            const long long off = a.cand_off[q], cap = a.cand_off[q + 1] - off;
            const int basep = sh->base;
            for (int i = tid; i < cnt; i += NT)
                if (basep + i < cap) a.cand[off + basep + i] = sh->cbuf[i];
        }
        g = gend;
        q++;
    }
}

struct PairScanArgs {
    const uint8_t* codes; const long long* blk_off; const int* list_len;
    const int* pl_cnt; const int* pl_off; const unsigned long long* units; const unsigned* entries; const DphPairWork* work; int* next_unit;
    const unsigned short* lutq; const float2* qparams; const float* cd; const unsigned* gdense;
    unsigned* gthr; unsigned long long* cand; const long long* cand_off; int* cand_cnt;
    long long list_lo, list_hi; int nprobe; int keep;
    const DphUnit* udesc;
    unsigned one;
};
#define PCAP 1536
struct PairShared {
    unsigned long long cbuf[2][PCAP];
    SelectScratch sc;
    int cnt[2]; unsigned thr[2]; int base[2]; int ndone; int ndone_snap; int unit;
};
template <int IMM> __device__ __forceinline__ unsigned lds_imm_u32(unsigned addr) {
    unsigned v;
    asm volatile("ld.shared.u32 %0, [%1+%2];" : "=r"(v) : "r"(addr), "n"(IMM));
    return v;
}
template <int T0> __device__ __forceinline__ void pair_word(unsigned wv, unsigned y, unsigned& a0, unsigned& a1, unsigned& a2, unsigned& a3) {
    constexpr int TB = DPH_DYN_SMEM_BASE + (T0 >> 5) * 65536 + (T0 & 31) * 4;
    a0 += lds_imm_u32<TB + 0>(__byte_perm(wv, y, 0x7504));
    a1 += lds_imm_u32<TB + 4>(__byte_perm(wv, y, 0x7514));
    a2 += lds_imm_u32<TB + 8>(__byte_perm(wv, y, 0x7524));
    a3 += lds_imm_u32<TB + 12>(__byte_perm(wv, y, 0x7534));
}
template <int C> __device__ __forceinline__ void pair_chunk(const uint4& v, unsigned y, unsigned& a0, unsigned& a1, unsigned& a2, unsigned& a3) {
    pair_word<C * 16 + 0>(v.x, y, a0, a1, a2, a3);
    pair_word<C * 16 + 4>(v.y, y, a0, a1, a2, a3);
    pair_word<C * 16 + 8>(v.z, y, a0, a1, a2, a3);
    pair_word<C * 16 + 12>(v.w, y, a0, a1, a2, a3);
}
template <int CAP>
__device__ __forceinline__ void compact_buffer(unsigned long long* cb, int* cnt, unsigned* thr, int keep, unsigned* gthr_q, SelectScratch* sc) {
    const int tid = threadIdx.x;
    const int n = *cnt;
    unsigned long long pivot = block_radix_select([&](int i) { return cb[i]; }, n, keep, sc);
    constexpr int PER = (CAP + NT - 1) / NT;
    unsigned long long mine[PER];
#pragma unroll
    for (int e = 0; e < PER; e++) { int i = tid + e * NT; mine[e] = (i < n) ? cb[i] : 0ull; }
    __syncthreads();
    if (tid == 0) *cnt = 0;
    __syncthreads();
#pragma unroll
    for (int e = 0; e < PER; e++)
        if (mine[e] >= pivot && mine[e] != 0ull) { int p = atomicAdd(cnt, 1); cb[p] = mine[e]; }
    if (tid == 0) {
        unsigned t = (unsigned)(pivot >> 32);
        unsigned old = atomicMax(gthr_q, t);
        *thr = t > old ? t : old;
    }
    __syncthreads();
}
__device__ __forceinline__ void warp_append(bool pass, unsigned long long key, unsigned long long* cb, int* cnt, int cap, int lane) {
    const unsigned pm = __ballot_sync(0xffffffffu, pass);
    if (pm) {
        int basep = 0;
        if (lane == 0) basep = atomicAdd(cnt, __popc(pm));
        basep = __shfl_sync(0xffffffffu, basep, 0);
        if (pass) { int p = basep + __popc(pm & ((1u << lane) - 1u)); if (p < cap) cb[p] = key; }
    }
}

__global__ void __launch_bounds__(NT, 1) scan_pair_kernel(PairScanArgs a) {
    unsigned char* const smem = dph_smem;
    PairShared* sh = reinterpret_cast<PairShared*>(smem + SMEM_LUT_FAST);
    const int tid = threadIdx.x, lane = tid & 31, warp = tid >> 5;
    const int total_units = a.work->total_units;
    const unsigned segb = (unsigned)a.work->per;
    const unsigned ywin = (((unsigned)__cvta_generic_to_shared(dph_smem)) & 0xFF000000u) | ((unsigned)lane * 4u);

    while (true) {
        if (tid == 0) sh->unit = atomicAdd(a.next_unit, 1);
        __syncthreads();
        const int u = sh->unit;
        if (u >= total_units) break;
        const unsigned long long ud = a.units[u];
        const long long l = (long long)(ud & 0xFFFFFFFFull);
        const int it = (int)((ud >> 32) & 0xFFFFull);
        const int len = a.list_len[l];
        const unsigned nb = (unsigned)((len + 31) >> 5);
        const unsigned bi0 = (unsigned)(ud >> 48) * segb;
        const unsigned bend = (nb - bi0 < segb) ? nb : bi0 + segb;
        const int e0 = a.pl_off[l] + 2 * it;
        const bool has_b = (2 * it + 1) < a.pl_cnt[l];
        const unsigned ea = a.entries[e0], eb = has_b ? a.entries[e0 + 1] : ea;
        const long long qa = ea >> 10, qb = eb >> 10;
        const int ra = (int)(ea & 1023u), rb = (int)(eb & 1023u);
        __syncthreads();
        {
            const uint4* A4 = reinterpret_cast<const uint4*>(a.lutq + (size_t)qa * DPH_LUT_SCAN_FLOATS);
            const uint4* B4 = reinterpret_cast<const uint4*>(a.lutq + (size_t)qb * DPH_LUT_SCAN_FLOATS);
            uint4* dst = reinterpret_cast<uint4*>(smem);
            for (int i = tid; i < DPH_LUT_SCAN_FLOATS / 8; i += NT) {
                const uint4 va = __ldg(A4 + i);
                uint4 vb = make_uint4(0u, 0u, 0u, 0u);
                if (has_b) vb = __ldg(B4 + i);
                uint4 o0, o1;
                o0.x = (va.x & 0xFFFFu) | (vb.x << 16); o0.y = (va.x >> 16) | (vb.x & 0xFFFF0000u);
                o0.z = (va.y & 0xFFFFu) | (vb.y << 16); o0.w = (va.y >> 16) | (vb.y & 0xFFFF0000u);
                o1.x = (va.z & 0xFFFFu) | (vb.z << 16); o1.y = (va.z >> 16) | (vb.z & 0xFFFF0000u);
                o1.z = (va.w & 0xFFFFu) | (vb.w << 16); o1.w = (va.w >> 16) | (vb.w & 0xFFFF0000u);
                dst[2 * i] = o0; dst[2 * i + 1] = o1;
            }
        }
        if (tid == 0) {
            sh->cnt[0] = 0; sh->cnt[1] = 0; sh->ndone = 0; sh->ndone_snap = 0;
            sh->thr[0] = *((volatile unsigned*)(a.gthr + qa));
            sh->thr[1] = has_b ? *((volatile unsigned*)(a.gthr + qb)) : 0xFFFFFFFFu;
        }
        __syncthreads();
        const float2 pa = a.qparams[qa], pb = a.qparams[qb];
        const float base_a = a.cd[qa * a.nprobe + ra] + pa.y, base_b = a.cd[qb * a.nprobe + rb] + pb.y;
        const unsigned gs_a = a.gdense[qa * a.nprobe + ra], gs_b = a.gdense[qb * a.nprobe + rb];
        const uint4* lbase = reinterpret_cast<const uint4*>(a.codes + a.blk_off[l] * DPH_BLK_BYTES);

        unsigned b = bi0 + warp, bp = bi0 + warp;
        uint4 nxt[6];
#pragma unroll 1
        for (int r = 0; r < DPH_L2_PREFETCH_ROUNDS && bp < bend; r++, bp += NW)
            if (lane == 0) l2_prefetch_block(lbase + (size_t)bp * (DPH_BLK_BYTES / 16));
        bool more = b < bend;
        if (more) {
            const uint4* p = lbase + (size_t)b * (DPH_BLK_BYTES / 16) + lane;
#pragma unroll
            for (int c6 = 0; c6 < 6; c6++) nxt[c6] = ldg_stream(p + c6 * 32);
        }
        bool counted = false;
        while (true) {
            while (more) {
                if (*((volatile int*)&sh->cnt[0]) > PCAP - NT || *((volatile int*)&sh->cnt[1]) > PCAP - NT) break;
                uint4 cur[6];
#pragma unroll
                for (int c6 = 0; c6 < 6; c6++) cur[c6] = nxt[c6];
                const unsigned bcur = b;
                if (bp < bend) { if (lane == 0) l2_prefetch_block(lbase + (size_t)bp * (DPH_BLK_BYTES / 16)); bp += NW; }
                b += NW;
                more = b < bend;
                if (more) {
                    const uint4* p = lbase + (size_t)b * (DPH_BLK_BYTES / 16) + lane;
#pragma unroll
                    for (int c6 = 0; c6 < 6; c6++) nxt[c6] = ldg_stream(p + c6 * 32);
                }
                unsigned s0 = 0, s1 = 0, s2 = 0, s3 = 0;
                pair_chunk<0>(cur[0], ywin, s0, s1, s2, s3);
                pair_chunk<1>(cur[1], ywin, s0, s1, s2, s3);
                pair_chunk<2>(cur[2], ywin, s0, s1, s2, s3);
                pair_chunk<3>(cur[3], ywin, s0, s1, s2, s3);
                pair_chunk<4>(cur[4], ywin, s0, s1, s2, s3);
                pair_chunk<5>(cur[5], ywin, s0, s1, s2, s3);
                const unsigned tot = (s0 + s1) + (s2 + s3);
                const float sc_a = fmaf(pa.x, (float)(tot & 0xFFFFu), base_a);
                const float sc_b = fmaf(pb.x, (float)(tot >> 16), base_b);
                const unsigned j = bcur * 32u + lane;
                const bool valid = (int)j < len;
                const unsigned ka = dph_fkey(sc_a), kb = dph_fkey(sc_b);
                warp_append(valid && ka >= *((volatile unsigned*)&sh->thr[0]), ((unsigned long long)ka << 32) | (unsigned long long)(0xFFFFFFFFu - (gs_a + j)),
                            sh->cbuf[0], &sh->cnt[0], PCAP, lane);
                warp_append(valid && kb >= *((volatile unsigned*)&sh->thr[1]), ((unsigned long long)kb << 32) | (unsigned long long)(0xFFFFFFFFu - (gs_b + j)),
                            sh->cbuf[1], &sh->cnt[1], PCAP, lane);
            }
            if (!more && !counted) { counted = true; if (lane == 0) atomicAdd(&sh->ndone, 1); }
            __syncthreads();
            if (sh->cnt[0] > a.keep) compact_buffer<PCAP>(sh->cbuf[0], &sh->cnt[0], &sh->thr[0], a.keep, a.gthr + qa, &sh->sc);
            if (sh->cnt[1] > a.keep) compact_buffer<PCAP>(sh->cbuf[1], &sh->cnt[1], &sh->thr[1], a.keep, a.gthr + qb, &sh->sc);
            if (tid == 0) {
                unsigned ga = *((volatile unsigned*)(a.gthr + qa));
                if (ga > sh->thr[0]) sh->thr[0] = ga;
                if (has_b) { unsigned gb = *((volatile unsigned*)(a.gthr + qb)); if (gb > sh->thr[1]) sh->thr[1] = gb; }
                sh->ndone_snap = sh->ndone;
            }
            __syncthreads();
            if (sh->ndone_snap == NW) break;
        }
        for (int s2i = 0; s2i < (has_b ? 2 : 1); s2i++) {
            const long long q = s2i ? qb : qa;
            const int cnt = sh->cnt[s2i];
            if (tid == 0) sh->base[s2i] = atomicAdd(a.cand_cnt + q, cnt);
            __syncthreads();
            const long long off = a.cand_off[q], cap = a.cand_off[q + 1] - off;
            const int basep = sh->base[s2i];
            for (int i = tid; i < cnt; i += NT)
                if (basep + i < cap) a.cand[off + basep + i] = sh->cbuf[s2i][i];
        }
    }
}


#define QCAP 768
struct QuadShared {
    unsigned long long cbuf[4][QCAP];
    SelectScratch sc;
    DphUnit desc[2];
    int cnt[4]; unsigned thr[4]; int base[4]; int ndone; int ndone_snap; int unit; int full;
    long long qs[4];
};
__device__ __forceinline__ unsigned imad_add(unsigned x, unsigned one, unsigned c) {
    unsigned d;
    asm("mad.lo.u32 %0, %1, %2, %3;" : "=r"(d) : "r"(x), "r"(one), "r"(c));
    return d;
}
template <int T0, int IMADL> __device__ __forceinline__ void quad_word(unsigned wv, unsigned y, unsigned one, unsigned (&sr)[4], unsigned (&ab)[4]) {
    constexpr int TB = DPH_DYN_SMEM_BASE + (T0 >> 5) * 65536 + (T0 & 31) * 4;
    constexpr int A = (T0 >> 2) & 1;
    const unsigned w0 = lds_imm_u32<TB + 0>(__byte_perm(wv, y, 0x7504));
    const unsigned w1 = lds_imm_u32<TB + 4>(__byte_perm(wv, y, 0x7514));
    const unsigned w2 = lds_imm_u32<TB + 8>(__byte_perm(wv, y, 0x7524));
    const unsigned w3 = lds_imm_u32<TB + 12>(__byte_perm(wv, y, 0x7534));
    if (IMADL >= 1) {
        sr[2 * A] = imad_add(w1, one, imad_add(w0, one, sr[2 * A]));
        sr[2 * A + 1] = imad_add(w3, one, imad_add(w2, one, sr[2 * A + 1]));
    } else {
        sr[2 * A] += w0 + w1;
        sr[2 * A + 1] += w2 + w3;
    }
    const unsigned e0 = __byte_perm(w0, 0u, 0x4341), e1 = __byte_perm(w1, 0u, 0x4341);
    const unsigned e2 = __byte_perm(w2, 0u, 0x4341), e3 = __byte_perm(w3, 0u, 0x4341);
    if (IMADL >= 3 || (IMADL == 2 && A == 1)) {
        ab[2 * A] = imad_add(e1, one, imad_add(e0, one, ab[2 * A]));
        ab[2 * A + 1] = imad_add(e3, one, imad_add(e2, one, ab[2 * A + 1]));
    } else {
        ab[2 * A] += e0 + e1;
        ab[2 * A + 1] += e2 + e3;
    }
}
template <int C, int IMADL> __device__ __forceinline__ void quad_chunk(const uint4& v, unsigned y, unsigned one, unsigned (&sr)[4], unsigned (&ab)[4]) {
    quad_word<C * 16 + 0, IMADL>(v.x, y, one, sr, ab);
    quad_word<C * 16 + 4, IMADL>(v.y, y, one, sr, ab);
    quad_word<C * 16 + 8, IMADL>(v.z, y, one, sr, ab);
    quad_word<C * 16 + 12, IMADL>(v.w, y, one, sr, ab);
}
__device__ __forceinline__ void warp_append_latch(bool pass, unsigned long long key, unsigned long long* cb, int* cnt, int* full, int lane) {
    const unsigned pm = __ballot_sync(0xffffffffu, pass);
    if (pm) {
        int basep = 0;
        const int np = __popc(pm);
        if (lane == 0) { basep = atomicAdd(cnt, np); if (basep + np > QCAP - NT) *((volatile int*)full) = 1; }
        basep = __shfl_sync(0xffffffffu, basep, 0);
        if (pass) { int p = basep + __popc(pm & ((1u << lane) - 1u)); if (p < QCAP) cb[p] = key; }
    }
}
__device__ __forceinline__ void cp_async16(void* smem_dst, const void* gsrc) {
    asm volatile("cp.async.ca.shared.global [%0], [%1], 16;" :: "r"((unsigned)__cvta_generic_to_shared(smem_dst)), "l"(gsrc) : "memory");
}

template <int IMADL>
__global__ void __launch_bounds__(NT, 1) scan_quad_kernel(PairScanArgs a) {
    unsigned char* const smem = dph_smem;
    QuadShared* sh = reinterpret_cast<QuadShared*>(smem + SMEM_LUT_FAST);
    const int tid = threadIdx.x, lane = tid & 31, warp = tid >> 5;
    const int total_units = a.work->total_units;
    const unsigned ywin = (((unsigned)__cvta_generic_to_shared(dph_smem)) & 0xFF000000u) | ((unsigned)lane * 4u);
    const unsigned char* lut8 = reinterpret_cast<const unsigned char*>(a.lutq);
    const unsigned one = a.one;

    if (tid == 0) sh->unit = atomicAdd(a.next_unit, 1);
    __syncthreads();
    {
        const int u = sh->unit;
        if (u >= total_units) return;
        if (tid < (int)(sizeof(DphUnit) / 16)) reinterpret_cast<uint4*>(&sh->desc[0])[tid] = __ldg(reinterpret_cast<const uint4*>(a.udesc + u) + tid);
    }
    __syncthreads();
    int cur = 0;
    while (true) {
        int next_u = 0;
        if (tid == 0) next_u = atomicAdd(a.next_unit, 1);
        const DphUnit* dsc = &sh->desc[cur];
        const int len = dsc->len, nq = dsc->nq;
        const unsigned bi0 = dsc->bi0, bend = dsc->bend;
        const uint4* lbase = reinterpret_cast<const uint4*>(a.codes + dsc->blk * DPH_BLK_BYTES);
        unsigned qv[4], gsv[4]; float stepv[4], basev[4];
#pragma unroll
        for (int i = 0; i < 4; i++) { qv[i] = dsc->q[i]; gsv[i] = dsc->gs[i]; basev[i] = dsc->base[i]; stepv[i] = dsc->step[i]; }

        unsigned b = bi0 + warp, bp = bi0 + warp;
        uint4 nxt[6];
#pragma unroll 1
        for (int r = 0; r < DPH_L2_PREFETCH_ROUNDS && bp < bend; r++, bp += NW)
            if (lane == 0) l2_prefetch_block(lbase + (size_t)bp * (DPH_BLK_BYTES / 16));
        bool more = b < bend;
        if (more) {
            const uint4* p = lbase + (size_t)b * (DPH_BLK_BYTES / 16) + lane;
#pragma unroll
            for (int c6 = 0; c6 < 6; c6++) nxt[c6] = ldg_stream(p + c6 * 32);
        }
        unsigned g4[4] = {0u, 0u, 0u, 0u};
        if (tid == 0) {
#pragma unroll
            for (int i = 0; i < 4; i++) g4[i] = i < nq ? *((volatile unsigned*)(a.gthr + qv[i])) : 0xFFFFFFFFu;
        }
        {
            const unsigned* T0p = reinterpret_cast<const unsigned*>(lut8 + (size_t)qv[0] * DPH_LUT_SCAN_FLOATS);
            const unsigned* T1p = reinterpret_cast<const unsigned*>(lut8 + (size_t)qv[1] * DPH_LUT_SCAN_FLOATS);
            const unsigned* T2p = reinterpret_cast<const unsigned*>(lut8 + (size_t)qv[2] * DPH_LUT_SCAN_FLOATS);
            const unsigned* T3p = reinterpret_cast<const unsigned*>(lut8 + (size_t)qv[3] * DPH_LUT_SCAN_FLOATS);
            uint4* dst = reinterpret_cast<uint4*>(smem);
            constexpr int LB = 6;
#pragma unroll 1
            for (int i0 = tid; i0 < 768 * 8; i0 += NT * LB) {
                unsigned va[LB], vb[LB], vc[LB], vd[LB];
#pragma unroll
                for (int e = 0; e < LB; e++) {
                    const int i = i0 + e * NT, src = (i >> 3) * 16 + (i & 7);
                    va[e] = __ldg(T0p + src); vb[e] = __ldg(T1p + src); vc[e] = __ldg(T2p + src); vd[e] = __ldg(T3p + src);
                }
#pragma unroll
                for (int e = 0; e < LB; e++) {
                    const int i = i0 + e * NT, row = i >> 3, cg = i & 7;
                    const unsigned t0 = __byte_perm(va[e], vb[e], 0x5140), t1 = __byte_perm(va[e], vb[e], 0x7362);
                    const unsigned u0 = __byte_perm(vc[e], vd[e], 0x5140), u1 = __byte_perm(vc[e], vd[e], 0x7362);
                    uint4 o;
                    o.x = __byte_perm(t0, u0, 0x5410); o.y = __byte_perm(t0, u0, 0x7632);
                    o.z = __byte_perm(t1, u1, 0x5410); o.w = __byte_perm(t1, u1, 0x7632);
                    dst[row * 16 + cg] = o;
                    dst[row * 16 + 8 + cg] = o;
                }
            }
        }
        if (tid == 0) {
            sh->ndone = 0; sh->ndone_snap = 0; sh->full = 0;
#pragma unroll
            for (int i = 0; i < 4; i++) { sh->cnt[i] = 0; sh->qs[i] = (long long)qv[i]; sh->thr[i] = g4[i]; }
        }
        __syncthreads();
        if (warp == 0) {
            const int nu = __shfl_sync(0xffffffffu, next_u, 0);
            if (lane == 0) sh->unit = nu;
            if (nu < total_units && lane < (int)(sizeof(DphUnit) / 16))
                cp_async16(reinterpret_cast<unsigned char*>(&sh->desc[cur ^ 1]) + lane * 16, reinterpret_cast<const unsigned char*>(a.udesc + nu) + lane * 16);
            asm volatile("cp.async.commit_group;" ::: "memory");
        }
        unsigned thr0 = sh->thr[0], thr1 = sh->thr[1], thr2 = sh->thr[2], thr3 = sh->thr[3];
        auto thr_f = [](unsigned t) { return t == 0xFFFFFFFFu ? __int_as_float(0x7f800000) : (t == 0u ? -__int_as_float(0x7f800000) : dph_fkey_inv(t)); };
        float tf0 = thr_f(thr0), tf1 = thr_f(thr1), tf2 = thr_f(thr2), tf3 = thr_f(thr3);

        bool counted = false;
        while (true) {
            while (more) {
                if (*((volatile int*)&sh->full)) break;
                uint4 cur6[6];
#pragma unroll
                for (int c6 = 0; c6 < 6; c6++) cur6[c6] = nxt[c6];
                const unsigned bcur = b;
                if (bp < bend) { if (lane == 0) l2_prefetch_block(lbase + (size_t)bp * (DPH_BLK_BYTES / 16)); bp += NW; }
                b += NW;
                more = b < bend;
                if (more) {
                    const uint4* p = lbase + (size_t)b * (DPH_BLK_BYTES / 16) + lane;
#pragma unroll
                    for (int c6 = 0; c6 < 6; c6++) nxt[c6] = ldg_stream(p + c6 * 32);
                }
                unsigned sr[4] = {0u, 0u, 0u, 0u}, ab[4] = {0u, 0u, 0u, 0u};
                quad_chunk<0, IMADL>(cur6[0], ywin, one, sr, ab);
                quad_chunk<1, IMADL>(cur6[1], ywin, one, sr, ab);
                quad_chunk<2, IMADL>(cur6[2], ywin, one, sr, ab);
                quad_chunk<3, IMADL>(cur6[3], ywin, one, sr, ab);
                quad_chunk<4, IMADL>(cur6[4], ywin, one, sr, ab);
                quad_chunk<5, IMADL>(cur6[5], ywin, one, sr, ab);
                const unsigned SR = (sr[0] + sr[1]) + (sr[2] + sr[3]);
                const unsigned AB = (ab[0] + ab[1]) + (ab[2] + ab[3]);
                const unsigned AE = SR - (AB << 8);
                const unsigned j = bcur * 32u + lane;
                const bool valid = (int)j < len;
                const float f0 = fmaf(stepv[0], (float)(unsigned short)(AE), basev[0]);
                const float f1 = fmaf(stepv[1], (float)(unsigned short)(AB), basev[1]);
                const float f2 = fmaf(stepv[2], (float)(unsigned short)(AE >> 16), basev[2]);
                const float f3 = fmaf(stepv[3], (float)(unsigned short)(AB >> 16), basev[3]);
                const bool p0 = valid && f0 >= tf0, p1 = valid && f1 >= tf1, p2 = valid && f2 >= tf2, p3 = valid && f3 >= tf3;
                if (__any_sync(0xffffffffu, p0 || p1 || p2 || p3)) {
                    const unsigned k0 = dph_fkey(f0), k1 = dph_fkey(f1), k2 = dph_fkey(f2), k3 = dph_fkey(f3);
                    warp_append_latch(p0 && k0 >= thr0, ((unsigned long long)k0 << 32) | (unsigned long long)(0xFFFFFFFFu - (gsv[0] + j)), sh->cbuf[0], &sh->cnt[0], &sh->full, lane);
                    warp_append_latch(p1 && k1 >= thr1, ((unsigned long long)k1 << 32) | (unsigned long long)(0xFFFFFFFFu - (gsv[1] + j)), sh->cbuf[1], &sh->cnt[1], &sh->full, lane);
                    warp_append_latch(p2 && k2 >= thr2, ((unsigned long long)k2 << 32) | (unsigned long long)(0xFFFFFFFFu - (gsv[2] + j)), sh->cbuf[2], &sh->cnt[2], &sh->full, lane);
                    warp_append_latch(p3 && k3 >= thr3, ((unsigned long long)k3 << 32) | (unsigned long long)(0xFFFFFFFFu - (gsv[3] + j)), sh->cbuf[3], &sh->cnt[3], &sh->full, lane);
                }
            }
            if (!more && !counted) { counted = true; if (lane == 0) atomicAdd(&sh->ndone, 1); }
            __syncthreads();
#pragma unroll 1
            for (int i = 0; i < nq; i++)
                if (sh->cnt[i] > a.keep) compact_buffer<QCAP>(sh->cbuf[i], &sh->cnt[i], &sh->thr[i], a.keep, a.gthr + sh->qs[i], &sh->sc);
            if (tid == 0) {
                for (int i = 0; i < nq; i++) { unsigned g = *((volatile unsigned*)(a.gthr + sh->qs[i])); if (g > sh->thr[i]) sh->thr[i] = g; }
                sh->ndone_snap = sh->ndone;
                sh->full = 0;
            }
            __syncthreads();
            thr0 = sh->thr[0]; thr1 = sh->thr[1]; thr2 = sh->thr[2]; thr3 = sh->thr[3];
            tf0 = thr_f(thr0); tf1 = thr_f(thr1); tf2 = thr_f(thr2); tf3 = thr_f(thr3);
            if (sh->ndone_snap == NW) break;
        }
        if (tid < nq) sh->base[tid] = atomicAdd(a.cand_cnt + sh->qs[tid], sh->cnt[tid]);
        if (warp == 0) asm volatile("cp.async.wait_all;" ::: "memory");
        __syncthreads();
#pragma unroll 1
        for (int i = 0; i < nq; i++) {
            const long long q = sh->qs[i];
            const int cnt = sh->cnt[i];
            const long long off = a.cand_off[q], cap = a.cand_off[q + 1] - off;
            const int basep = sh->base[i];
            for (int c = tid; c < cnt; c += NT)
                if (basep + c < cap) a.cand[off + basep + c] = sh->cbuf[i][c];
        }
        const int un = sh->unit;
        __syncthreads();
        if (un >= total_units) break;
        cur ^= 1;
    }
}

__global__ void smem_base_probe_kernel(unsigned* out) { *out = (unsigned)__cvta_generic_to_shared(dph_smem) & 0x00FFFFFFu; }

int dph_scan_setup_attrs() {
    static DphPerDeviceOnce once;
    if (!once.first()) return 0;
    {
        unsigned* d = nullptr; unsigned h = 0;
        DPH_CUDA(cudaMalloc((void**)&d, 4));
        smem_base_probe_kernel<<<1, 32, 1024>>>(d);
        DPH_CUDA(cudaMemcpy(&h, d, 4, cudaMemcpyDeviceToHost));
        cudaFree(d);
        DPH_CHECK(h == DPH_DYN_SMEM_BASE, "dynamic shared memory window does not start at 0x400 on this driver; rebuild with the probed value");
    }
    DPH_CUDA(cudaFuncSetAttribute(scan_kernel<DPH_SCAN_FAST>, cudaFuncAttributeMaxDynamicSharedMemorySize, SMEM_LUT_FAST + (int)sizeof(ScanShared)));
    DPH_CUDA(cudaFuncSetAttribute(scan_kernel<DPH_SCAN_EXACT>, cudaFuncAttributeMaxDynamicSharedMemorySize, SMEM_LUT_EXACT + (int)sizeof(ScanShared)));
    DPH_CUDA(cudaFuncSetAttribute(scan_pair_kernel, cudaFuncAttributeMaxDynamicSharedMemorySize, SMEM_LUT_FAST + (int)sizeof(PairShared)));
    DPH_CUDA(cudaFuncSetAttribute(scan_quad_kernel<0>, cudaFuncAttributeMaxDynamicSharedMemorySize, SMEM_LUT_FAST + (int)sizeof(QuadShared)));
    DPH_CUDA(cudaFuncSetAttribute(scan_quad_kernel<1>, cudaFuncAttributeMaxDynamicSharedMemorySize, SMEM_LUT_FAST + (int)sizeof(QuadShared)));
    DPH_CUDA(cudaFuncSetAttribute(scan_quad_kernel<2>, cudaFuncAttributeMaxDynamicSharedMemorySize, SMEM_LUT_FAST + (int)sizeof(QuadShared)));
    DPH_CUDA(cudaFuncSetAttribute(scan_quad_kernel<3>, cudaFuncAttributeMaxDynamicSharedMemorySize, SMEM_LUT_FAST + (int)sizeof(QuadShared)));
    return 0;
}

int dph_launch_scan(dph_index* ix, int64_t n, int k, int keep, int mode, int grid, cudaStream_t st) {
    (void)k;
    if (n == 0) return 0;
    DPH_TRY(dph_scan_setup_attrs());
    ScanArgs a;
    a.codes = ix->codes; a.qpre = ix->wpre.as<long long>(); a.segs = ix->segs.as<DphSeg>(); a.nseg = ix->nseg.as<int>(); a.work = ix->work.as<DphWork>();
    a.lut_canon = ix->lut_canon.as<float>(); a.gthr = ix->gthr.as<unsigned>();
    a.cand = ix->cand.as<unsigned long long>(); a.cand_off = ix->cand_off.as<long long>(); a.cand_cnt = ix->cand_cnt.as<int>();
    a.n = n; a.nprobe = ix->nprobe; a.keep = keep;
    if (mode == DPH_SCAN_FAST)
        scan_kernel<DPH_SCAN_FAST><<<grid, NT, SMEM_LUT_FAST + sizeof(ScanShared), st>>>(a);
    else
        scan_kernel<DPH_SCAN_EXACT><<<grid, NT, SMEM_LUT_EXACT + sizeof(ScanShared), st>>>(a);
    DPH_CUDA(cudaGetLastError());
    return 0;
}

int dph_launch_scan_pair(dph_index* ix, int64_t n, int keep, int grid, cudaStream_t st, int group) {
    if (n == 0) return 0;
    DPH_TRY(dph_scan_setup_attrs());
    PairScanArgs a;
    a.codes = ix->codes; a.blk_off = (const long long*)ix->blk_off; a.list_len = ix->list_len; a.pl_cnt = ix->pl_cnt.as<int>();
    a.pl_off = ix->pl_off.as<int>(); a.units = ix->pl_units.as<unsigned long long>(); a.entries = ix->pl_entries.as<unsigned>();
    a.work = ix->pairwork.as<DphPairWork>(); a.next_unit = &ix->pairwork.as<DphPairWork>()->next_unit; a.lutq = ix->lutq.as<unsigned short>(); a.qparams = ix->qparams.as<float2>();
    a.cd = ix->cd.as<float>(); a.gdense = ix->gdense.as<unsigned>(); a.gthr = ix->gthr.as<unsigned>();
    a.cand = ix->cand.as<unsigned long long>(); a.cand_off = ix->cand_off.as<long long>(); a.cand_cnt = ix->cand_cnt.as<int>();
    a.list_lo = ix->list_lo; a.list_hi = ix->list_hi; a.nprobe = ix->nprobe; a.keep = keep;
    a.udesc = ix->pl_udesc.as<DphUnit>(); a.one = 1u;
    if (group == 4) {
        const size_t sm = SMEM_LUT_FAST + sizeof(QuadShared);
        switch (g_dph_tune[0]) {
            case 0: scan_quad_kernel<0><<<grid, NT, sm, st>>>(a); break;
            case 2: scan_quad_kernel<2><<<grid, NT, sm, st>>>(a); break;
            case 3: scan_quad_kernel<3><<<grid, NT, sm, st>>>(a); break;
            default: scan_quad_kernel<1><<<grid, NT, sm, st>>>(a); break;
        }
    }
    else scan_pair_kernel<<<grid, NT, SMEM_LUT_FAST + sizeof(PairShared), st>>>(a);
    DPH_CUDA(cudaGetLastError());
    return 0;
}

struct MergeArgs {
    const unsigned long long* cand; const long long* cand_off; const int* cand_cnt; const unsigned* gthr; const float* eps;
    const DphSeg* segs; const int* nseg; int nprobe; int k; int mode;
    const uint8_t* codes; const float* lut_canon; const long long* ids; const long long* list_start;
    float* D; long long* I; unsigned* G; int* flags; const int* only_flagged;
};

__device__ __forceinline__ int find_seg(const unsigned* gstart, int nsg, unsigned gidx) {
    int lo = 0, hi = nsg;
    while (hi - lo > 1) { int mid = (lo + hi) >> 1; if (gstart[mid] <= gidx) lo = mid; else hi = mid; }
    return lo;
}

__global__ void __launch_bounds__(256) merge_kernel(MergeArgs a) {
    __shared__ SelectScratch sc;
    __shared__ unsigned long long surv[DPH_SURV_CAP];
    __shared__ unsigned sgs[DPH_MAX_NPROBE];
    __shared__ int scnt, sflag;
    const long long q = blockIdx.x;
    const int tid = threadIdx.x;
    if (a.only_flagged && a.only_flagged[q] == 0) return;
    const unsigned long long* E = a.cand + a.cand_off[q];
    long long cap = a.cand_off[q + 1] - a.cand_off[q];
    int n = a.cand_cnt[q];
    const bool overflow = n > cap;
    if (n > cap) n = (int)cap;
    const DphSeg* segs = a.segs + q * a.nprobe;
    const int nsg = a.nseg[q];
    const int k = a.k;
    if (tid == 0) { scnt = 0; sflag = 0; }
    for (int i = tid; i < nsg; i += blockDim.x) sgs[i] = segs[i].gstart;
    __syncthreads();
    auto get = [&](int i) { return E[i]; };
    unsigned long long pivot = 0ull;
    int flag = overflow ? 1 : 0;
    if (a.mode == DPH_SCAN_FAST) {
        const float eps2 = 2.0f * a.eps[q];
        const unsigned gt = a.gthr[q];
        if (n > k) {
            unsigned long long pk = block_radix_select(get, n, k, &sc);
            const float Tk = dph_ckey_score(pk);
            if (gt != 0u && !(Tk - dph_fkey_inv(gt) > eps2)) flag = 1;
            pivot = (unsigned long long)dph_fkey(Tk - eps2) << 32;
        } else if (gt != 0u) flag = 1;
    } else {
        if (n > DPH_SURV_CAP) pivot = block_radix_select(get, n, k, &sc);
    }
    for (int i = tid; i < n; i += blockDim.x) {
        unsigned long long e = E[i];
        if (e >= pivot) { int p = atomicAdd(&scnt, 1); if (p < DPH_SURV_CAP) surv[p] = e; else sflag = 1; }
    }
    __syncthreads();
    int ns = scnt < DPH_SURV_CAP ? scnt : DPH_SURV_CAP;
    if (sflag) flag = 1;
    if (a.mode == DPH_SCAN_FAST) {
        const float* lutc = a.lut_canon + (size_t)q * DPH_LUT_CANON_FLOATS;
        const int lane = tid & 31, warp = tid >> 5, nwarps = blockDim.x >> 5;
        for (int i = warp; i < ns; i += nwarps) {
            const unsigned gidx = dph_ckey_gidx(surv[i]);
            const DphSeg s = segs[find_seg(sgs, nsg, gidx)];
            const unsigned j = gidx - s.gstart;
            const uint8_t* blk = a.codes + (s.blk + (long long)(j >> 5)) * DPH_BLK_BYTES;
            const int ln = (int)(j & 31u);
            float v[3];
#pragma unroll
            for (int h = 0; h < 3; h++) {
                const int m = h * 32 + lane;
                v[h] = __ldg(lutc + DPH_LUTC_IDX(m, (int)blk[dph_blk_addr(ln, m)]));
            }
            float dis = s.dis0;
#pragma unroll
            for (int h = 0; h < 3; h++)
#pragma unroll
                for (int l2 = 0; l2 < 32; l2++) dis += __shfl_sync(0xffffffffu, v[h], l2);
            __syncwarp();
            if (lane == 0) surv[i] = dph_ckey(dis, gidx);
        }
    }
    const int p2 = dph_next_pow2(ns > 1 ? ns : 1);
    for (int i = ns + tid; i < p2; i += blockDim.x) surv[i] = 0ull;
    __syncthreads();
    block_bitonic_sort_desc(surv, p2);
    for (int i = tid; i < k; i += blockDim.x) {
        float d = DPH_NEUTRAL; long long id = -1; unsigned gi = 0xFFFFFFFFu;
        if (i < ns) {
            const unsigned long long e = surv[i];
            gi = dph_ckey_gidx(e); d = dph_ckey_score(e);
            const DphSeg s = segs[find_seg(sgs, nsg, gi)];
            const unsigned j = gi - s.gstart;
            id = a.ids ? a.ids[s.blk * 32 + j] : a.list_start[s.list] + (long long)j;
        }
        a.D[q * k + i] = d; a.I[q * k + i] = id; a.G[q * k + i] = gi;
    }
    if (a.mode == DPH_SCAN_FAST && tid == 0) a.flags[q] = flag;
}

int dph_launch_merge(dph_index* ix, int64_t n, int k, int mode, const int32_t* only_flagged, float* D, int64_t* I, uint32_t* G,
                     cudaStream_t st) {
    if (n == 0) return 0;
    MergeArgs a;
    a.cand = ix->cand.as<unsigned long long>(); a.cand_off = ix->cand_off.as<long long>(); a.cand_cnt = ix->cand_cnt.as<int>();
    a.gthr = ix->gthr.as<unsigned>(); a.eps = ix->eps.as<float>(); a.segs = ix->segs.as<DphSeg>(); a.nseg = ix->nseg.as<int>(); a.nprobe = ix->nprobe; a.k = k; a.mode = mode;
    a.codes = ix->codes; a.lut_canon = ix->lut_canon.as<float>(); a.ids = (const long long*)ix->ids; a.list_start = (const long long*)ix->list_start;
    a.D = D; a.I = (long long*)I; a.G = G; a.flags = ix->flags.as<int>(); a.only_flagged = only_flagged;
    merge_kernel<<<(unsigned)n, 256, 0, st>>>(a);
    DPH_CUDA(cudaGetLastError());
    return 0;
}

__global__ void pack_topk_kernel(const float* D, const long long* I, const unsigned* G, long long total, longlong2* P) {
    long long i = (long long)blockIdx.x * blockDim.x + threadIdx.x;
    if (i >= total) return;
    longlong2 v;
    v.x = I[i] >= 0 ? (long long)dph_ckey(D[i], G[i]) : 0ll;
    v.y = I[i];
    P[i] = v;
}
__global__ void __launch_bounds__(256) merge_packed_kernel(const longlong2* Pg, int nshards, long long n, int k, float* D, long long* I) {
    extern __shared__ unsigned long long mp[];
    const long long q = blockIdx.x;
    const int tot = nshards * k, p2 = dph_next_pow2(tot);
    unsigned long long* keys = mp;
    for (int i = threadIdx.x; i < p2; i += blockDim.x) {
        unsigned long long key = 0ull;
        if (i < tot) key = (unsigned long long)Pg[((long long)(i / k) * n + q) * k + (i % k)].x;
        keys[i] = key;
    }
    __syncthreads();
    block_bitonic_sort_desc(keys, p2);
    for (int i = threadIdx.x; i < k; i += blockDim.x) {
        float d = DPH_NEUTRAL; long long id = -1;
        const unsigned long long key = keys[i];
        if (key != 0ull) {
            d = dph_ckey_score(key);
            for (int j = 0; j < tot && id < 0; j++) {
                const longlong2 e = Pg[((long long)(j / k) * n + q) * k + (j % k)];
                if ((unsigned long long)e.x == key) id = e.y;
            }
        }
        D[q * k + i] = d; I[q * k + i] = id;
    }
}
DPH_API int dph_pack_topk(const float* D, const int64_t* I, const uint32_t* G, int64_t n, int k, int64_t* P, void* cuda_stream) {
    const long long total = (long long)n * k;
    if (total == 0) return 0;
    pack_topk_kernel<<<(unsigned)((total + 255) / 256), 256, 0, (cudaStream_t)cuda_stream>>>(D, (const long long*)I, G, total, (longlong2*)P);
    DPH_CUDA(cudaGetLastError());
    return 0;
}
DPH_API int dph_merge_shards_packed(const int64_t* Pg, int nshards, int64_t n, int k, float* D, int64_t* I, void* cuda_stream) {
    if (n == 0) return 0;
    DPH_CHECK(nshards >= 1 && k >= 1 && (long long)nshards * k <= 8192, "merge_shards: nshards*k must be <= 8192");
    int p2 = 1; while (p2 < nshards * k) p2 <<= 1;
    static DphPerDeviceOnce once;
    if (once.first()) { DPH_CUDA(cudaFuncSetAttribute(merge_packed_kernel, cudaFuncAttributeMaxDynamicSharedMemorySize, 8192 * 8)); }
    merge_packed_kernel<<<(unsigned)n, 256, p2 * 8, (cudaStream_t)cuda_stream>>>((const longlong2*)Pg, nshards, n, k, D, (long long*)I);
    DPH_CUDA(cudaGetLastError());
    return 0;
}

__global__ void __launch_bounds__(256) merge_shards_kernel(const float* Dg, const long long* Ig, const unsigned* Gg, int nshards, long long n,
                                                            int k, float* D, long long* I) {
    extern __shared__ unsigned long long ms[];
    const long long q = blockIdx.x;
    const int tid = threadIdx.x;
    const int tot = nshards * k;
    const int p2 = dph_next_pow2(tot);
    unsigned long long* keys = ms;
    for (int i = tid; i < p2; i += blockDim.x) {
        unsigned long long key = 0ull;
        if (i < tot) {
            int s = i / k, r = i % k;
            long long id = Ig[((long long)s * n + q) * k + r];
            if (id >= 0) key = dph_ckey(Dg[((long long)s * n + q) * k + r], Gg[((long long)s * n + q) * k + r]);
        }
        keys[i] = key;
    }
    __syncthreads();
    block_bitonic_sort_desc(keys, p2);
    for (int i = tid; i < k; i += blockDim.x) {
        float d = DPH_NEUTRAL; long long id = -1;
        unsigned long long key = keys[i];
        if (key != 0ull) {
            unsigned gi = dph_ckey_gidx(key);
            d = dph_ckey_score(key);
            for (int s = 0; s < nshards && id < 0; s++)
                for (int r = 0; r < k; r++) {
                    long long o = ((long long)s * n + q) * k + r;
                    if (Gg[o] == gi && Ig[o] >= 0) { id = Ig[o]; break; }
                }
        }
        D[q * k + i] = d; I[q * k + i] = id;
    }
}

DPH_API int dph_merge_shards(const float* Dg, const int64_t* Ig, const uint32_t* Gg, int nshards, int64_t n, int k, float* D, int64_t* I,
                                void* cuda_stream) {
    if (n == 0) return 0;
    DPH_CHECK(nshards >= 1 && k >= 1 && (long long)nshards * k <= 8192, "merge_shards: nshards*k must be <= 8192");
    int p2 = 1; while (p2 < nshards * k) p2 <<= 1;
    static DphPerDeviceOnce once;
    if (once.first()) { DPH_CUDA(cudaFuncSetAttribute(merge_shards_kernel, cudaFuncAttributeMaxDynamicSharedMemorySize, 8192 * 8)); }
    merge_shards_kernel<<<(unsigned)n, 256, p2 * 8, (cudaStream_t)cuda_stream>>>(Dg, (const long long*)Ig, Gg, nshards, n, k, D, (long long*)I);
    DPH_CUDA(cudaGetLastError());
    return 0;
}
```

Before: 15600.

## Scan up to eight queries per code block in quad kernel with packed dual tables

Raises the number of queries served per pass over a list's code blocks from four to eight. Each code byte is now gathered from two packed 16-bit LUT tables using rotation-based addressing, and the block runs with 256 threads, a smaller per-query candidate buffer and fewer L2 prefetch rounds. The aim is to amortize global code loads across more queries when lists are shared. In exchange, each block issues more shared-memory gathers per code, has less buffer headroom so compaction happens more often, and carries a larger unit descriptor; optional phase-timing instrumentation is also added.

Result: faster. 18780 (median of 6 runs) (+20.4%).

```diff
diff --git a/densephrases_b200/csrc/common.cuh b/densephrases_b200/csrc/common.cuh
--- a/densephrases_b200/csrc/common.cuh
+++ b/densephrases_b200/csrc/common.cuh
@@ -114,16 +114,17 @@
     int total_units;
     int next_unit;
 };
+#define DPH_QUAD_ITEM_Q 8
 struct __align__(16) DphUnit {
     long long blk;
     int len;
     unsigned bi0, bend;
     int nq;
     int list, pad;
-    unsigned q[4];
-    unsigned gs[4];
-    float base[4];
-    float step[4];
+    unsigned q[DPH_QUAD_ITEM_Q];
+    unsigned gs[DPH_QUAD_ITEM_Q];
+    float base[DPH_QUAD_ITEM_Q];
+    float step[DPH_QUAD_ITEM_Q];
 };
 #define DPH_PAIR_SEG_MIN 128
 #define DPH_PAIR_UNITS_PER_CTA 16
diff --git a/densephrases_b200/csrc/index.cu b/densephrases_b200/csrc/index.cu
--- a/densephrases_b200/csrc/index.cu
+++ b/densephrases_b200/csrc/index.cu
@@ -624,7 +624,8 @@
     if (group == 2 && keep_pair > 1536 - DPH_SCAN_THREADS) group = 1;
     const bool pair = group > 1;
     const int keep_fast = group == 4 ? keep_quad : (group == 2 ? keep_pair : keep_single);
-    DPH_TRY(ix->cand.ensure(((size_t)(2 * grid + 2 * n + 2) + (pair ? (size_t)(n * nprobe + 2 * DPH_PAIR_UNITS_PER_CTA * grid + 2 * n + 16) : 0)) * keep_max * 8));
+    const size_t item_q = group == 4 ? DPH_QUAD_ITEM_Q : 2;
+    DPH_TRY(ix->cand.ensure(((size_t)(2 * grid + 2 * n + 2) + (pair ? (size_t)(n * nprobe + item_q * DPH_PAIR_UNITS_PER_CTA * grid + 2 * n + 16) : 0)) * keep_max * 8));
     DPH_TRY(ix->cand_off.ensure((size_t)(n + 1) * 8));
     DPH_TRY(ix->cand_cnt.ensure((size_t)n * 4));
     DPH_TRY(ix->gthr.ensure((size_t)n * 4));
diff --git a/densephrases_b200/csrc/index_internal.cuh b/densephrases_b200/csrc/index_internal.cuh
--- a/densephrases_b200/csrc/index_internal.cuh
+++ b/densephrases_b200/csrc/index_internal.cuh
@@ -20,7 +20,7 @@
 #define DPH_LUT_CANON_FLOATS (96 * 256)
 #define DPH_LUTC_IDX(m, code) ((((m) >> 5) << 13) + ((code) << 5) + ((m) & 31))
 #define DPH_SEG_SMEM 256
-#define DPH_L2_PREFETCH_ROUNDS 4
+#define DPH_L2_PREFETCH_ROUNDS 2
 
 struct DevBuf {
     void* p = nullptr;
diff --git a/densephrases_b200/csrc/prep.cu b/densephrases_b200/csrc/prep.cu
--- a/densephrases_b200/csrc/prep.cu
+++ b/densephrases_b200/csrc/prep.cu
@@ -845,10 +845,10 @@
         DphUnit d;
         if (a.udesc) {
             d.blk = a.blk_off[l]; d.len = a.list_len[l]; d.list = (int)l; d.pad = 0;
-            d.nq = min(4, cnt - 4 * it);
-            const int e0 = a.off[l] + 4 * it;
-#pragma unroll
-            for (int i = 0; i < 4; i++) {
+            d.nq = min(a.gsz, cnt - a.gsz * it);
+            const int e0 = a.off[l] + a.gsz * it;
+#pragma unroll
+            for (int i = 0; i < DPH_QUAD_ITEM_Q; i++) {
                 const unsigned e = a.entries[e0 + (i < d.nq ? i : 0)];
                 const long long q = e >> 10; const int r = (int)(e & 1023u);
                 const float2 pp = a.qparams[q];
@@ -894,7 +894,7 @@
         p.list_hi = ix->list_hi; p.nlist = ix->nlist; p.grid = grid; p.cnt = ix->pl_cnt.as<int>(); p.fill = ix->pl_fill.as<int>();
         p.off = ix->pl_off.as<int>(); p.blockpre = ix->pl_blockpre.as<long long>(); p.entries = ix->pl_entries.as<unsigned>();
         p.work = ix->pairwork.as<DphPairWork>(); p.unitpre = ix->pl_unitpre.as<int>(); p.units = ix->pl_units.as<unsigned long long>();
-        p.gsz = group;
+        p.gsz = group == 4 ? DPH_QUAD_ITEM_Q : group;
         p.udesc = group == 4 ? ix->pl_udesc.as<DphUnit>() : nullptr;
         p.blk_off = (const long long*)ix->blk_off; p.cd = ix->cd.as<float>(); p.gdense = ix->gdense.as<unsigned>(); p.qparams = ix->qparams.as<float2>();
         DPH_CUDA(cudaMemsetAsync(p.cnt, 0, (size_t)ix->nlist * 4, st));
diff --git a/densephrases_b200/csrc/scan.cu b/densephrases_b200/csrc/scan.cu
--- a/densephrases_b200/csrc/scan.cu
+++ b/densephrases_b200/csrc/scan.cu
@@ -290,15 +290,15 @@
     pair_word<C * 16 + 8>(v.z, y, a0, a1, a2, a3);
     pair_word<C * 16 + 12>(v.w, y, a0, a1, a2, a3);
 }
-template <int CAP>
+template <int CAP, int NTH>
 __device__ __forceinline__ void compact_buffer(unsigned long long* cb, int* cnt, unsigned* thr, int keep, unsigned* gthr_q, SelectScratch* sc) {
     const int tid = threadIdx.x;
     const int n = *cnt;
     unsigned long long pivot = block_radix_select([&](int i) { return cb[i]; }, n, keep, sc);
-    constexpr int PER = (CAP + NT - 1) / NT;
+    constexpr int PER = (CAP + NTH - 1) / NTH;
     unsigned long long mine[PER];
 #pragma unroll
-    for (int e = 0; e < PER; e++) { int i = tid + e * NT; mine[e] = (i < n) ? cb[i] : 0ull; }
+    for (int e = 0; e < PER; e++) { int i = tid + e * NTH; mine[e] = (i < n) ? cb[i] : 0ull; }
     __syncthreads();
     if (tid == 0) *cnt = 0;
     __syncthreads();
@@ -422,8 +422,8 @@
             }
             if (!more && !counted) { counted = true; if (lane == 0) atomicAdd(&sh->ndone, 1); }
             __syncthreads();
-            if (sh->cnt[0] > a.keep) compact_buffer<PCAP>(sh->cbuf[0], &sh->cnt[0], &sh->thr[0], a.keep, a.gthr + qa, &sh->sc);
-            if (sh->cnt[1] > a.keep) compact_buffer<PCAP>(sh->cbuf[1], &sh->cnt[1], &sh->thr[1], a.keep, a.gthr + qb, &sh->sc);
+            if (sh->cnt[0] > a.keep) compact_buffer<PCAP, NT>(sh->cbuf[0], &sh->cnt[0], &sh->thr[0], a.keep, a.gthr + qa, &sh->sc);
+            if (sh->cnt[1] > a.keep) compact_buffer<PCAP, NT>(sh->cbuf[1], &sh->cnt[1], &sh->thr[1], a.keep, a.gthr + qb, &sh->sc);
             if (tid == 0) {
                 unsigned ga = *((volatile unsigned*)(a.gthr + qa));
                 if (ga > sh->thr[0]) sh->thr[0] = ga;
@@ -447,26 +447,31 @@
 }
 
 
-#define QCAP 768
+#define QNT 256
+#define QNW (QNT / 32)
+#define QCAP 512
+#define SMEM_QUAD_TABLES (3 * 65536)
+static_assert(QCAP - QNT == DPH_QUAD_KEEP_MAX, "quad latch margin");
 struct QuadShared {
-    unsigned long long cbuf[4][QCAP];
+    unsigned long long cbuf[DPH_QUAD_ITEM_Q][QCAP];
     SelectScratch sc;
     DphUnit desc[2];
-    int cnt[4]; unsigned thr[4]; int base[4]; int ndone; int ndone_snap; int unit; int full;
-    long long qs[4];
+    int cnt[DPH_QUAD_ITEM_Q]; unsigned thr[DPH_QUAD_ITEM_Q]; int base[DPH_QUAD_ITEM_Q]; int ndone; int ndone_snap; int unit; int full;
+    long long qs[DPH_QUAD_ITEM_Q];
 };
 __device__ __forceinline__ unsigned imad_add(unsigned x, unsigned one, unsigned c) {
     unsigned d;
     asm("mad.lo.u32 %0, %1, %2, %3;" : "=r"(d) : "r"(x), "r"(one), "r"(c));
     return d;
 }
-template <int T0, int IMADL> __device__ __forceinline__ void quad_word(unsigned wv, unsigned y, unsigned one, unsigned (&sr)[4], unsigned (&ab)[4]) {
-    constexpr int TB = DPH_DYN_SMEM_BASE + (T0 >> 5) * 65536 + (T0 & 31) * 4;
+template <int T0, int TAB, int IMADL> __device__ __forceinline__ void quad_gather(const unsigned (&ad)[4], unsigned one, unsigned (&sr)[4], unsigned (&ab)[4]) {
+    constexpr int S = T0 >> 5;
+    constexpr int TB = DPH_DYN_SMEM_BASE + (S < 2 ? TAB : 2) * 65536 + (S < 2 ? S : TAB) * 128;
     constexpr int A = (T0 >> 2) & 1;
-    const unsigned w0 = lds_imm_u32<TB + 0>(__byte_perm(wv, y, 0x7504));
-    const unsigned w1 = lds_imm_u32<TB + 4>(__byte_perm(wv, y, 0x7514));
-    const unsigned w2 = lds_imm_u32<TB + 8>(__byte_perm(wv, y, 0x7524));
-    const unsigned w3 = lds_imm_u32<TB + 12>(__byte_perm(wv, y, 0x7534));
+    const unsigned w0 = lds_imm_u32<TB>(ad[0]);
+    const unsigned w1 = lds_imm_u32<TB>(ad[1]);
+    const unsigned w2 = lds_imm_u32<TB>(ad[2]);
+    const unsigned w3 = lds_imm_u32<TB>(ad[3]);
     if (IMADL >= 1) {
         sr[2 * A] = imad_add(w1, one, imad_add(w0, one, sr[2 * A]));
         sr[2 * A + 1] = imad_add(w3, one, imad_add(w2, one, sr[2 * A + 1]));
@@ -484,18 +489,29 @@
         ab[2 * A + 1] += e2 + e3;
     }
 }
-template <int C, int IMADL> __device__ __forceinline__ void quad_chunk(const uint4& v, unsigned y, unsigned one, unsigned (&sr)[4], unsigned (&ab)[4]) {
-    quad_word<C * 16 + 0, IMADL>(v.x, y, one, sr, ab);
-    quad_word<C * 16 + 4, IMADL>(v.y, y, one, sr, ab);
-    quad_word<C * 16 + 8, IMADL>(v.z, y, one, sr, ab);
-    quad_word<C * 16 + 12, IMADL>(v.w, y, one, sr, ab);
+template <int T> struct RotSel { static constexpr int reg = (T & 31) / 3, sel = 0x7700 | (4 + (T & 31) % 3); };
+template <int T0, int NTAB, int IMADL> __device__ __forceinline__ void quad_word(unsigned wv, const unsigned (&rot)[11], unsigned one,
+                                                                                  unsigned (&sr)[2][4], unsigned (&ab)[2][4]) {
+    const unsigned ad[4] = {__byte_perm(wv, rot[RotSel<T0>::reg], RotSel<T0>::sel | 0x00),
+                            __byte_perm(wv, rot[RotSel<T0 + 1>::reg], RotSel<T0 + 1>::sel | 0x10),
+                            __byte_perm(wv, rot[RotSel<T0 + 2>::reg], RotSel<T0 + 2>::sel | 0x20),
+                            __byte_perm(wv, rot[RotSel<T0 + 3>::reg], RotSel<T0 + 3>::sel | 0x30)};
+    quad_gather<T0, 0, IMADL>(ad, one, sr[0], ab[0]);
+    if (NTAB == 2) quad_gather<T0, 1, IMADL>(ad, one, sr[1], ab[1]);
+}
+template <int C, int NTAB, int IMADL> __device__ __forceinline__ void quad_chunk(const uint4& v, const unsigned (&rot)[11], unsigned one,
+                                                                                   unsigned (&sr)[2][4], unsigned (&ab)[2][4]) {
+    quad_word<C * 16 + 0, NTAB, IMADL>(v.x, rot, one, sr, ab);
+    quad_word<C * 16 + 4, NTAB, IMADL>(v.y, rot, one, sr, ab);
+    quad_word<C * 16 + 8, NTAB, IMADL>(v.z, rot, one, sr, ab);
+    quad_word<C * 16 + 12, NTAB, IMADL>(v.w, rot, one, sr, ab);
 }
 __device__ __forceinline__ void warp_append_latch(bool pass, unsigned long long key, unsigned long long* cb, int* cnt, int* full, int lane) {
     const unsigned pm = __ballot_sync(0xffffffffu, pass);
     if (pm) {
         int basep = 0;
         const int np = __popc(pm);
-        if (lane == 0) { basep = atomicAdd(cnt, np); if (basep + np > QCAP - NT) *((volatile int*)full) = 1; }
+        if (lane == 0) { basep = atomicAdd(cnt, np); if (basep + np > QCAP - QNT) *((volatile int*)full) = 1; }
         basep = __shfl_sync(0xffffffffu, basep, 0);
         if (pass) { int p = basep + __popc(pm & ((1u << lane) - 1u)); if (p < QCAP) cb[p] = key; }
     }
@@ -503,87 +519,186 @@
 __device__ __forceinline__ void cp_async16(void* smem_dst, const void* gsrc) {
     asm volatile("cp.async.ca.shared.global [%0], [%1], 16;" :: "r"((unsigned)__cvta_generic_to_shared(smem_dst)), "l"(gsrc) : "memory");
 }
+__device__ __forceinline__ float quad_thr_f(unsigned t) {
+    return t == 0xFFFFFFFFu ? __int_as_float(0x7f800000) : (t == 0u ? -__int_as_float(0x7f800000) : dph_fkey_inv(t));
+}
+
+#ifdef DPH_SCAN_PHASES
+__device__ unsigned long long g_quad_phase_ns[4];
+__device__ unsigned g_quad_phase_ctas;
+__device__ __forceinline__ unsigned long long globaltimer_ns() { unsigned long long t; asm volatile("mov.u64 %0, %globaltimer;" : "=l"(t)); return t; }
+#define QPH_MARK(i) do { if (threadIdx.x == 0) { const unsigned long long t_ = globaltimer_ns(); ph[i] += t_ - ph_t; ph_t = t_; } } while (0)
+#else
+#define QPH_MARK(i) do { } while (0)
+#endif
+
+template <int NTAB, int IMADL>
+__device__ __forceinline__ void quad_item_rounds(const PairScanArgs& a, QuadShared* sh, const DphUnit* dsc, const uint4* lbase, unsigned b,
+                                                 unsigned bp, uint4 (&nxt)[6], const unsigned (&rot)[11], unsigned one, unsigned long long* ph,
+                                                 unsigned long long& ph_t) {
+    (void)ph; (void)ph_t;
+    const int lane = threadIdx.x & 31;
+    const int len = dsc->len, nq = dsc->nq;
+    const unsigned bend = dsc->bend;
+    constexpr int NS = 4 * NTAB;
+    unsigned gsv[NS]; float stepv[NS], basev[NS], tf[NS]; unsigned thr[NS];
+#pragma unroll
+    for (int i = 0; i < NS; i++) { gsv[i] = dsc->gs[i]; basev[i] = dsc->base[i]; stepv[i] = dsc->step[i]; thr[i] = sh->thr[i]; tf[i] = quad_thr_f(thr[i]); }
+    bool more = b < bend, counted = false;
+    while (true) {
+        while (more) {
+            if (*((volatile int*)&sh->full)) break;
+            uint4 cur6[6];
+#pragma unroll
+            for (int c6 = 0; c6 < 6; c6++) cur6[c6] = nxt[c6];
+            const unsigned bcur = b;
+            if (bp < bend) { if (lane == 0) l2_prefetch_block(lbase + (size_t)bp * (DPH_BLK_BYTES / 16)); bp += QNW; }
+            b += QNW;
+            more = b < bend;
+            if (more) {
+                const uint4* p = lbase + (size_t)b * (DPH_BLK_BYTES / 16) + lane;
+#pragma unroll
+                for (int c6 = 0; c6 < 6; c6++) nxt[c6] = ldg_stream(p + c6 * 32);
+            }
+            unsigned sr[2][4] = {}, ab[2][4] = {};
+            quad_chunk<0, NTAB, IMADL>(cur6[0], rot, one, sr, ab);
+            quad_chunk<1, NTAB, IMADL>(cur6[1], rot, one, sr, ab);
+            quad_chunk<2, NTAB, IMADL>(cur6[2], rot, one, sr, ab);
+            quad_chunk<3, NTAB, IMADL>(cur6[3], rot, one, sr, ab);
+            quad_chunk<4, NTAB, IMADL>(cur6[4], rot, one, sr, ab);
+            quad_chunk<5, NTAB, IMADL>(cur6[5], rot, one, sr, ab);
+            const unsigned j = bcur * 32u + lane;
+            const bool valid = (int)j < len;
+            float f[NS]; bool p[NS]; bool any = false;
+#pragma unroll
+            for (int tb = 0; tb < NTAB; tb++) {
+                const unsigned SR = (sr[tb][0] + sr[tb][1]) + (sr[tb][2] + sr[tb][3]);
+                const unsigned AB = (ab[tb][0] + ab[tb][1]) + (ab[tb][2] + ab[tb][3]);
+                const unsigned AE = SR - (AB << 8);
+                f[4 * tb + 0] = fmaf(stepv[4 * tb + 0], (float)(unsigned short)(AE), basev[4 * tb + 0]);
+                f[4 * tb + 1] = fmaf(stepv[4 * tb + 1], (float)(unsigned short)(AB), basev[4 * tb + 1]);
+                f[4 * tb + 2] = fmaf(stepv[4 * tb + 2], (float)(unsigned short)(AE >> 16), basev[4 * tb + 2]);
+                f[4 * tb + 3] = fmaf(stepv[4 * tb + 3], (float)(unsigned short)(AB >> 16), basev[4 * tb + 3]);
+            }
+#pragma unroll
+            for (int i = 0; i < NS; i++) { p[i] = valid && f[i] >= tf[i]; any = any || p[i]; }
+            if (__any_sync(0xffffffffu, any)) {
+#pragma unroll
+                for (int i = 0; i < NS; i++) {
+                    const unsigned k = dph_fkey(f[i]);
+                    warp_append_latch(p[i] && k >= thr[i], ((unsigned long long)k << 32) | (unsigned long long)(0xFFFFFFFFu - (gsv[i] + j)),
+                                      sh->cbuf[i], &sh->cnt[i], &sh->full, lane);
+                }
+            }
+        }
+        if (!more && !counted) { counted = true; if (lane == 0) atomicAdd(&sh->ndone, 1); }
+        __syncthreads();
+        QPH_MARK(1);
+#pragma unroll 1
+        for (int i = 0; i < nq; i++)
+            if (sh->cnt[i] > a.keep) compact_buffer<QCAP, QNT>(sh->cbuf[i], &sh->cnt[i], &sh->thr[i], a.keep, a.gthr + sh->qs[i], &sh->sc);
+        if (threadIdx.x == 0) {
+            for (int i = 0; i < nq; i++) { unsigned g = *((volatile unsigned*)(a.gthr + sh->qs[i])); if (g > sh->thr[i]) sh->thr[i] = g; }
+            sh->ndone_snap = sh->ndone;
+            sh->full = 0;
+        }
+        __syncthreads();
+        QPH_MARK(2);
+#pragma unroll
+        for (int i = 0; i < NS; i++) { thr[i] = sh->thr[i]; tf[i] = quad_thr_f(thr[i]); }
+        if (sh->ndone_snap == QNW) break;
+    }
+}
 
 template <int IMADL>
-__global__ void __launch_bounds__(NT, 1) scan_quad_kernel(PairScanArgs a) {
+__global__ void __launch_bounds__(QNT, 1) scan_quad_kernel(PairScanArgs a) {
     unsigned char* const smem = dph_smem;
-    QuadShared* sh = reinterpret_cast<QuadShared*>(smem + SMEM_LUT_FAST);
+    QuadShared* sh = reinterpret_cast<QuadShared*>(smem + SMEM_QUAD_TABLES);
     const int tid = threadIdx.x, lane = tid & 31, warp = tid >> 5;
     const int total_units = a.work->total_units;
-    const unsigned ywin = (((unsigned)__cvta_generic_to_shared(dph_smem)) & 0xFF000000u) | ((unsigned)lane * 4u);
     const unsigned char* lut8 = reinterpret_cast<const unsigned char*>(a.lutq);
     const unsigned one = a.one;
+    unsigned rot[11];
+#pragma unroll
+    for (int r = 0; r < 11; r++) {
+        unsigned v = 0;
+#pragma unroll
+        for (int bb = 0; bb < 3; bb++)
+            if (3 * r + bb < 32) v |= (unsigned)(((lane + 3 * r + bb) & 31) * 4) << (8 * bb);
+        rot[r] = v;
+    }
+    unsigned long long ph[4] = {0ull, 0ull, 0ull, 0ull}, ph_t = 0ull;
+#ifdef DPH_SCAN_PHASES
+    if (tid == 0) ph_t = globaltimer_ns();
+#endif
 
     if (tid == 0) sh->unit = atomicAdd(a.next_unit, 1);
     __syncthreads();
-    {
-        const int u = sh->unit;
-        if (u >= total_units) return;
-        if (tid < (int)(sizeof(DphUnit) / 16)) reinterpret_cast<uint4*>(&sh->desc[0])[tid] = __ldg(reinterpret_cast<const uint4*>(a.udesc + u) + tid);
-    }
-    __syncthreads();
     int cur = 0;
-    while (true) {
+    bool any_unit = sh->unit < total_units;
+    if (any_unit && tid < (int)(sizeof(DphUnit) / 16))
+        reinterpret_cast<uint4*>(&sh->desc[0])[tid] = __ldg(reinterpret_cast<const uint4*>(a.udesc + sh->unit) + tid);
+    __syncthreads();
+    while (any_unit) {
         int next_u = 0;
         if (tid == 0) next_u = atomicAdd(a.next_unit, 1);
         const DphUnit* dsc = &sh->desc[cur];
-        const int len = dsc->len, nq = dsc->nq;
+        const int nq = dsc->nq;
+        const int ntab = nq > 4 ? 2 : 1;
         const unsigned bi0 = dsc->bi0, bend = dsc->bend;
         const uint4* lbase = reinterpret_cast<const uint4*>(a.codes + dsc->blk * DPH_BLK_BYTES);
-        unsigned qv[4], gsv[4]; float stepv[4], basev[4];
-#pragma unroll
-        for (int i = 0; i < 4; i++) { qv[i] = dsc->q[i]; gsv[i] = dsc->gs[i]; basev[i] = dsc->base[i]; stepv[i] = dsc->step[i]; }
 
         unsigned b = bi0 + warp, bp = bi0 + warp;
         uint4 nxt[6];
 #pragma unroll 1
-        for (int r = 0; r < DPH_L2_PREFETCH_ROUNDS && bp < bend; r++, bp += NW)
+        for (int r = 0; r < DPH_L2_PREFETCH_ROUNDS && bp < bend; r++, bp += QNW)
             if (lane == 0) l2_prefetch_block(lbase + (size_t)bp * (DPH_BLK_BYTES / 16));
-        bool more = b < bend;
-        if (more) {
+        if (b < bend) {
             const uint4* p = lbase + (size_t)b * (DPH_BLK_BYTES / 16) + lane;
 #pragma unroll
             for (int c6 = 0; c6 < 6; c6++) nxt[c6] = ldg_stream(p + c6 * 32);
         }
-        unsigned g4[4] = {0u, 0u, 0u, 0u};
-        if (tid == 0) {
-#pragma unroll
-            for (int i = 0; i < 4; i++) g4[i] = i < nq ? *((volatile unsigned*)(a.gthr + qv[i])) : 0xFFFFFFFFu;
-        }
+        unsigned gq = 0xFFFFFFFFu;
+        if (tid < DPH_QUAD_ITEM_Q && tid < nq) gq = *((volatile unsigned*)(a.gthr + dsc->q[tid]));
         {
-            const unsigned* T0p = reinterpret_cast<const unsigned*>(lut8 + (size_t)qv[0] * DPH_LUT_SCAN_FLOATS);
-            const unsigned* T1p = reinterpret_cast<const unsigned*>(lut8 + (size_t)qv[1] * DPH_LUT_SCAN_FLOATS);
-            const unsigned* T2p = reinterpret_cast<const unsigned*>(lut8 + (size_t)qv[2] * DPH_LUT_SCAN_FLOATS);
-            const unsigned* T3p = reinterpret_cast<const unsigned*>(lut8 + (size_t)qv[3] * DPH_LUT_SCAN_FLOATS);
+            const unsigned* src[DPH_QUAD_ITEM_Q];
+#pragma unroll
+            for (int i = 0; i < DPH_QUAD_ITEM_Q; i++) src[i] = reinterpret_cast<const unsigned*>(lut8 + (size_t)dsc->q[i] * DPH_LUT_SCAN_FLOATS);
             uint4* dst = reinterpret_cast<uint4*>(smem);
-            constexpr int LB = 6;
+            constexpr int LB = 6, PER_TAB = 768 * 8;
+            static_assert(PER_TAB % (QNT * LB) == 0, "a batch of the build stays inside one table");
 #pragma unroll 1
-            for (int i0 = tid; i0 < 768 * 8; i0 += NT * LB) {
+            for (int i0 = tid; i0 < ntab * PER_TAB; i0 += QNT * LB) {
+                const int tb = i0 >= PER_TAB;
+                const unsigned* T0p = tb ? src[4] : src[0];
+                const unsigned* T1p = tb ? src[5] : src[1];
+                const unsigned* T2p = tb ? src[6] : src[2];
+                const unsigned* T3p = tb ? src[7] : src[3];
+                const int ib = i0 - tb * PER_TAB;
                 unsigned va[LB], vb[LB], vc[LB], vd[LB];
 #pragma unroll
                 for (int e = 0; e < LB; e++) {
-                    const int i = i0 + e * NT, src = (i >> 3) * 16 + (i & 7);
-                    va[e] = __ldg(T0p + src); vb[e] = __ldg(T1p + src); vc[e] = __ldg(T2p + src); vd[e] = __ldg(T3p + src);
+                    const int i = ib + e * QNT, s = (i >> 3) * 16 + (i & 7);
+                    va[e] = __ldg(T0p + s); vb[e] = __ldg(T1p + s); vc[e] = __ldg(T2p + s); vd[e] = __ldg(T3p + s);
                 }
 #pragma unroll
                 for (int e = 0; e < LB; e++) {
-                    const int i = i0 + e * NT, row = i >> 3, cg = i & 7;
+                    const int i = ib + e * QNT, row = i >> 3, cg = i & 7;
+                    const int seg = row >> 8, code = row & 255;
+                    const int region = seg < 2 ? tb : 2, half = seg < 2 ? seg : tb;
                     const unsigned t0 = __byte_perm(va[e], vb[e], 0x5140), t1 = __byte_perm(va[e], vb[e], 0x7362);
                     const unsigned u0 = __byte_perm(vc[e], vd[e], 0x5140), u1 = __byte_perm(vc[e], vd[e], 0x7362);
                     uint4 o;
                     o.x = __byte_perm(t0, u0, 0x5410); o.y = __byte_perm(t0, u0, 0x7632);
                     o.z = __byte_perm(t1, u1, 0x5410); o.w = __byte_perm(t1, u1, 0x7632);
-                    dst[row * 16 + cg] = o;
-                    dst[row * 16 + 8 + cg] = o;
+                    dst[region * 4096 + code * 16 + half * 8 + cg] = o;
                 }
             }
         }
-        if (tid == 0) {
-            sh->ndone = 0; sh->ndone_snap = 0; sh->full = 0;
-#pragma unroll
-            for (int i = 0; i < 4; i++) { sh->cnt[i] = 0; sh->qs[i] = (long long)qv[i]; sh->thr[i] = g4[i]; }
-        }
-        __syncthreads();
+        if (tid < DPH_QUAD_ITEM_Q) { sh->cnt[tid] = 0; sh->qs[tid] = (long long)dsc->q[tid]; sh->thr[tid] = gq; }
+        if (tid == 0) { sh->ndone = 0; sh->ndone_snap = 0; sh->full = 0; }
+        __syncthreads();
+        QPH_MARK(0);
         if (warp == 0) {
             const int nu = __shfl_sync(0xffffffffu, next_u, 0);
             if (lane == 0) sh->unit = nu;
@@ -591,66 +706,8 @@
                 cp_async16(reinterpret_cast<unsigned char*>(&sh->desc[cur ^ 1]) + lane * 16, reinterpret_cast<const unsigned char*>(a.udesc + nu) + lane * 16);
             asm volatile("cp.async.commit_group;" ::: "memory");
         }
-        unsigned thr0 = sh->thr[0], thr1 = sh->thr[1], thr2 = sh->thr[2], thr3 = sh->thr[3];
-        auto thr_f = [](unsigned t) { return t == 0xFFFFFFFFu ? __int_as_float(0x7f800000) : (t == 0u ? -__int_as_float(0x7f800000) : dph_fkey_inv(t)); };
-        float tf0 = thr_f(thr0), tf1 = thr_f(thr1), tf2 = thr_f(thr2), tf3 = thr_f(thr3);
-
-        bool counted = false;
-        while (true) {
-            while (more) {
-                if (*((volatile int*)&sh->full)) break;
-                uint4 cur6[6];
-#pragma unroll
-                for (int c6 = 0; c6 < 6; c6++) cur6[c6] = nxt[c6];
-                const unsigned bcur = b;
-                if (bp < bend) { if (lane == 0) l2_prefetch_block(lbase + (size_t)bp * (DPH_BLK_BYTES / 16)); bp += NW; }
-                b += NW;
-                more = b < bend;
-                if (more) {
-                    const uint4* p = lbase + (size_t)b * (DPH_BLK_BYTES / 16) + lane;
-#pragma unroll
-                    for (int c6 = 0; c6 < 6; c6++) nxt[c6] = ldg_stream(p + c6 * 32);
-                }
-                unsigned sr[4] = {0u, 0u, 0u, 0u}, ab[4] = {0u, 0u, 0u, 0u};
-                quad_chunk<0, IMADL>(cur6[0], ywin, one, sr, ab);
-                quad_chunk<1, IMADL>(cur6[1], ywin, one, sr, ab);
-                quad_chunk<2, IMADL>(cur6[2], ywin, one, sr, ab);
-                quad_chunk<3, IMADL>(cur6[3], ywin, one, sr, ab);
-                quad_chunk<4, IMADL>(cur6[4], ywin, one, sr, ab);
-                quad_chunk<5, IMADL>(cur6[5], ywin, one, sr, ab);
-                const unsigned SR = (sr[0] + sr[1]) + (sr[2] + sr[3]);
-                const unsigned AB = (ab[0] + ab[1]) + (ab[2] + ab[3]);
-                const unsigned AE = SR - (AB << 8);
-                const unsigned j = bcur * 32u + lane;
-                const bool valid = (int)j < len;
-                const float f0 = fmaf(stepv[0], (float)(unsigned short)(AE), basev[0]);
-                const float f1 = fmaf(stepv[1], (float)(unsigned short)(AB), basev[1]);
-                const float f2 = fmaf(stepv[2], (float)(unsigned short)(AE >> 16), basev[2]);
-                const float f3 = fmaf(stepv[3], (float)(unsigned short)(AB >> 16), basev[3]);
-                const bool p0 = valid && f0 >= tf0, p1 = valid && f1 >= tf1, p2 = valid && f2 >= tf2, p3 = valid && f3 >= tf3;
-                if (__any_sync(0xffffffffu, p0 || p1 || p2 || p3)) {
-                    const unsigned k0 = dph_fkey(f0), k1 = dph_fkey(f1), k2 = dph_fkey(f2), k3 = dph_fkey(f3);
-                    warp_append_latch(p0 && k0 >= thr0, ((unsigned long long)k0 << 32) | (unsigned long long)(0xFFFFFFFFu - (gsv[0] + j)), sh->cbuf[0], &sh->cnt[0], &sh->full, lane);
-                    warp_append_latch(p1 && k1 >= thr1, ((unsigned long long)k1 << 32) | (unsigned long long)(0xFFFFFFFFu - (gsv[1] + j)), sh->cbuf[1], &sh->cnt[1], &sh->full, lane);
-                    warp_append_latch(p2 && k2 >= thr2, ((unsigned long long)k2 << 32) | (unsigned long long)(0xFFFFFFFFu - (gsv[2] + j)), sh->cbuf[2], &sh->cnt[2], &sh->full, lane);
-                    warp_append_latch(p3 && k3 >= thr3, ((unsigned long long)k3 << 32) | (unsigned long long)(0xFFFFFFFFu - (gsv[3] + j)), sh->cbuf[3], &sh->cnt[3], &sh->full, lane);
-                }
-            }
-            if (!more && !counted) { counted = true; if (lane == 0) atomicAdd(&sh->ndone, 1); }
-            __syncthreads();
-#pragma unroll 1
-            for (int i = 0; i < nq; i++)
-                if (sh->cnt[i] > a.keep) compact_buffer<QCAP>(sh->cbuf[i], &sh->cnt[i], &sh->thr[i], a.keep, a.gthr + sh->qs[i], &sh->sc);
-            if (tid == 0) {
-                for (int i = 0; i < nq; i++) { unsigned g = *((volatile unsigned*)(a.gthr + sh->qs[i])); if (g > sh->thr[i]) sh->thr[i] = g; }
-                sh->ndone_snap = sh->ndone;
-                sh->full = 0;
-            }
-            __syncthreads();
-            thr0 = sh->thr[0]; thr1 = sh->thr[1]; thr2 = sh->thr[2]; thr3 = sh->thr[3];
-            tf0 = thr_f(thr0); tf1 = thr_f(thr1); tf2 = thr_f(thr2); tf3 = thr_f(thr3);
-            if (sh->ndone_snap == NW) break;
-        }
+        if (ntab == 2) quad_item_rounds<2, IMADL>(a, sh, dsc, lbase, b, bp, nxt, rot, one, ph, ph_t);
+        else quad_item_rounds<1, IMADL>(a, sh, dsc, lbase, b, bp, nxt, rot, one, ph, ph_t);
         if (tid < nq) sh->base[tid] = atomicAdd(a.cand_cnt + sh->qs[tid], sh->cnt[tid]);
         if (warp == 0) asm volatile("cp.async.wait_all;" ::: "memory");
         __syncthreads();
@@ -660,17 +717,32 @@
             const int cnt = sh->cnt[i];
             const long long off = a.cand_off[q], cap = a.cand_off[q + 1] - off;
             const int basep = sh->base[i];
-            for (int c = tid; c < cnt; c += NT)
+            for (int c = tid; c < cnt; c += QNT)
                 if (basep + c < cap) a.cand[off + basep + c] = sh->cbuf[i][c];
         }
-        const int un = sh->unit;
-        __syncthreads();
-        if (un >= total_units) break;
+        any_unit = sh->unit < total_units;
+        __syncthreads();
+        QPH_MARK(3);
         cur ^= 1;
     }
-}
-
-__global__ void smem_base_probe_kernel(unsigned* out) { *out = (unsigned)__cvta_generic_to_shared(dph_smem) & 0x00FFFFFFu; }
+#ifdef DPH_SCAN_PHASES
+    if (tid == 0) {
+        for (int i = 0; i < 4; i++) atomicAdd(&g_quad_phase_ns[i], ph[i]);
+        __threadfence();
+        if (atomicAdd(&g_quad_phase_ctas, 1u) == gridDim.x - 1) {
+            __threadfence();
+            unsigned long long v[4];
+            for (int i = 0; i < 4; i++) { v[i] = atomicExch(&g_quad_phase_ns[i], 0ull); }
+            printf("scan_quad_kernel phases (ms, summed over %u CTAs): table build %.3f, scan rounds %.3f, compaction barriers %.3f, publish %.3f\n",
+                   gridDim.x, v[0] * 1e-6, v[1] * 1e-6, v[2] * 1e-6, v[3] * 1e-6);
+            g_quad_phase_ctas = 0;
+        }
+    }
+#endif
+}
+#undef QPH_MARK
+
+__global__ void smem_base_probe_kernel(unsigned* out) { *out = (unsigned)__cvta_generic_to_shared(dph_smem); }
 
 int dph_scan_setup_attrs() {
     static DphPerDeviceOnce once;
@@ -686,10 +758,10 @@
     DPH_CUDA(cudaFuncSetAttribute(scan_kernel<DPH_SCAN_FAST>, cudaFuncAttributeMaxDynamicSharedMemorySize, SMEM_LUT_FAST + (int)sizeof(ScanShared)));
     DPH_CUDA(cudaFuncSetAttribute(scan_kernel<DPH_SCAN_EXACT>, cudaFuncAttributeMaxDynamicSharedMemorySize, SMEM_LUT_EXACT + (int)sizeof(ScanShared)));
     DPH_CUDA(cudaFuncSetAttribute(scan_pair_kernel, cudaFuncAttributeMaxDynamicSharedMemorySize, SMEM_LUT_FAST + (int)sizeof(PairShared)));
-    DPH_CUDA(cudaFuncSetAttribute(scan_quad_kernel<0>, cudaFuncAttributeMaxDynamicSharedMemorySize, SMEM_LUT_FAST + (int)sizeof(QuadShared)));
-    DPH_CUDA(cudaFuncSetAttribute(scan_quad_kernel<1>, cudaFuncAttributeMaxDynamicSharedMemorySize, SMEM_LUT_FAST + (int)sizeof(QuadShared)));
-    DPH_CUDA(cudaFuncSetAttribute(scan_quad_kernel<2>, cudaFuncAttributeMaxDynamicSharedMemorySize, SMEM_LUT_FAST + (int)sizeof(QuadShared)));
-    DPH_CUDA(cudaFuncSetAttribute(scan_quad_kernel<3>, cudaFuncAttributeMaxDynamicSharedMemorySize, SMEM_LUT_FAST + (int)sizeof(QuadShared)));
+    DPH_CUDA(cudaFuncSetAttribute(scan_quad_kernel<0>, cudaFuncAttributeMaxDynamicSharedMemorySize, SMEM_QUAD_TABLES + (int)sizeof(QuadShared)));
+    DPH_CUDA(cudaFuncSetAttribute(scan_quad_kernel<1>, cudaFuncAttributeMaxDynamicSharedMemorySize, SMEM_QUAD_TABLES + (int)sizeof(QuadShared)));
+    DPH_CUDA(cudaFuncSetAttribute(scan_quad_kernel<2>, cudaFuncAttributeMaxDynamicSharedMemorySize, SMEM_QUAD_TABLES + (int)sizeof(QuadShared)));
+    DPH_CUDA(cudaFuncSetAttribute(scan_quad_kernel<3>, cudaFuncAttributeMaxDynamicSharedMemorySize, SMEM_QUAD_TABLES + (int)sizeof(QuadShared)));
     return 0;
 }
 
@@ -722,12 +794,12 @@
     a.list_lo = ix->list_lo; a.list_hi = ix->list_hi; a.nprobe = ix->nprobe; a.keep = keep;
     a.udesc = ix->pl_udesc.as<DphUnit>(); a.one = 1u;
     if (group == 4) {
-        const size_t sm = SMEM_LUT_FAST + sizeof(QuadShared);
+        const size_t sm = SMEM_QUAD_TABLES + sizeof(QuadShared);
         switch (g_dph_tune[0]) {
-            case 0: scan_quad_kernel<0><<<grid, NT, sm, st>>>(a); break;
-            case 2: scan_quad_kernel<2><<<grid, NT, sm, st>>>(a); break;
-            case 3: scan_quad_kernel<3><<<grid, NT, sm, st>>>(a); break;
-            default: scan_quad_kernel<1><<<grid, NT, sm, st>>>(a); break;
+            case 0: scan_quad_kernel<0><<<grid, QNT, sm, st>>>(a); break;
+            case 2: scan_quad_kernel<2><<<grid, QNT, sm, st>>>(a); break;
+            case 3: scan_quad_kernel<3><<<grid, QNT, sm, st>>>(a); break;
+            default: scan_quad_kernel<1><<<grid, QNT, sm, st>>>(a); break;
         }
     }
     else scan_pair_kernel<<<grid, NT, SMEM_LUT_FAST + sizeof(PairShared), st>>>(a);
```
